# DearCaat/RRT-MIL

Hardware: AMD Instinct MI355X
Metric: slides/sec RRTEncoder fwd, N=9000 D=512 region_num=8 (higher is better)
Workload: dtype f32

## Files before the change

include/rrt_hip.h:

```cpp
#ifndef RRT_HIP_H
#define RRT_HIP_H
#include <stddef.h>
#include <stdint.h>

#ifdef __cplusplus
extern "C" {
#endif

#define RRT_ABI_VERSION 29
#define RRT_MAX_RMSA_LAYERS 8
#define RRT_MAX_CRMSA_K 8

enum {
  RRT_OK = 0,
  RRT_E_INVALID = -1,
  RRT_E_UNSUPPORTED = -2,
  RRT_E_WORKSPACE = -3,
  RRT_E_HANDOVER = -4
};

enum { RRT_COMPUTE_F32 = 0, RRT_COMPUTE_BF16 = 1, RRT_COMPUTE_F16 = 2, RRT_COMPUTE_F32X3 = 3 };
enum { RRT_POS_NONE = 0, RRT_POS_PEG = 1, RRT_POS_PPEG = 2 };
enum { RRT_EPEG_ATTN = 0, RRT_EPEG_VALUE_BF = 1, RRT_EPEG_VALUE_AF = 2 };

enum { RRT_ACT_NONE = 0, RRT_ACT_RELU = 1, RRT_ACT_GELU = 2, RRT_ACT_TANH = 3, RRT_ACT_SIGMOID = 4 };

typedef struct rrt_grid {
  int64_t L;
  int32_t H;
  int32_t s;
  int32_t regions_side;
  int64_t add;
} rrt_grid;

typedef struct rrt_encoder_desc {
  int32_t dim;
  int32_t n_heads;
  int32_t n_rmsa_layers;
  int32_t region_num;
  int32_t region_size;
  int32_t min_region_num;
  float   min_region_ratio;
  int32_t epeg;
  int32_t epeg_k;
  int32_t cr_msa;
  int32_t crmsa_k;
  int32_t crmsa_heads;
  int32_t crmsa_mlp;
  int32_t all_shortcut;
  int32_t compute;
  int32_t ffn;
  int32_t ffn_act;
  int32_t ffn_hidden;
  int32_t pos;
  int32_t pos_pos;
  int32_t peg_k;
  int32_t peg_1d;
  int32_t epeg_2d;
  int32_t epeg_type;
  int32_t weights16_valid;
  int32_t solo;
} rrt_encoder_desc;

typedef struct rrt_attn_weights {
  const float *norm_w, *norm_b;
  const float *qkv_w, *qkv_b;
  const float *proj_w, *proj_b;
  const float *pe_w, *pe_b;
  const float *norm2_w, *norm2_b;
  const float *fc1_w, *fc1_b;
  const float *fc2_w, *fc2_b;
} rrt_attn_weights;

typedef struct rrt_encoder_weights {
  rrt_attn_weights rmsa[RRT_MAX_RMSA_LAYERS];
  rrt_attn_weights crmsa;
  const float *phi;
  const float *phi0_w, *phi2_w;
  const float *norm_w, *norm_b;
  const float *pos_w[3], *pos_b[3];
  uint64_t version;
} rrt_encoder_weights;

int         rrt_abi_version(void);
const char *rrt_strerror(int code);

int rrt_region_grid(int64_t L, int32_t region_num, int32_t region_size,
                    int32_t min_region_num, float min_region_ratio, rrt_grid *out);

int rrt_encoder_workspace_size(const rrt_encoder_desc *desc, int64_t n_tokens, size_t *bytes);

#define RRT_PLAN_FUSED      1
#define RRT_PLAN_FUSED_PROJ 2
#define RRT_PLAN_FUSED16    4
#define RRT_PLAN_FUSED_X3   8
#define RRT_PLAN_CRMSA_PARTS 16
#define RRT_PLAN_ATTN_HD    32
int rrt_encoder_plan(const rrt_encoder_desc *desc, int64_t n_tokens, int32_t *flags);
int rrt_encoder_plan_rows(const rrt_encoder_desc *desc, int64_t n_tokens, int32_t *w);

int rrt_encoder_forward_f32(const rrt_encoder_desc *desc, const rrt_encoder_weights *w,
                            const float *x, float *y, int64_t n_tokens,
                            void *workspace, size_t workspace_bytes, void *stream);

int rrt_debug_encoder_forward_rows_f32(const rrt_encoder_desc *desc, const rrt_encoder_weights *w,
                                       const float *x, float *y, int64_t n_tokens,
                                       void *workspace, size_t workspace_bytes, void *stream, int32_t rows_w);

enum {
  RRT_EV_START = 0,
  RRT_EV_LN_PARTITION,
  RRT_EV_QKV,
  RRT_EV_ATTN,
  RRT_EV_PROJ,
  RRT_EV_CR_COMBINE,
  RRT_EV_CR_INNER,
  RRT_EV_END,
  RRT_EV_COUNT
};
int rrt_encoder_forward_events_f32(const rrt_encoder_desc *desc, const rrt_encoder_weights *w,
                                   const float *x, float *y, int64_t n_tokens,
                                   void *workspace, size_t workspace_bytes, void *stream,
                                   void **events);

typedef struct rrt_phase_gate rrt_phase_gate;
int rrt_phase_gate_create(rrt_phase_gate **out);
int rrt_phase_gate_destroy(rrt_phase_gate *gate);
int rrt_encoder_forward_gated_f32(const rrt_encoder_desc *desc, const rrt_encoder_weights *w,
                                  const float *x, float *y, int64_t n_tokens,
                                  void *workspace, size_t workspace_bytes, void *stream,
                                  rrt_phase_gate *gate, void **events);

int rrt_encoder_batch_workspace_size(const rrt_encoder_desc *desc, int32_t batch, int64_t n_tokens, size_t *bytes);
int rrt_encoder_forward_batch_f32(const rrt_encoder_desc *desc, const rrt_encoder_weights *w,
                                  const float *x, float *y, int32_t batch, int64_t n_tokens,
                                  void *workspace, size_t workspace_bytes, void *stream);


int rrt_ln_partition_f32(const float *x, const float *gamma, const float *beta, float *u,
                         int64_t L, int32_t dim, const rrt_grid *g, void *stream);

int rrt_ln_partition_rows_f32(const float *x, const float *gamma, const float *beta, float *u,
                              int64_t L, int32_t dim, const rrt_grid *g, int32_t w,
                              int32_t *zero, int32_t n_zero, void *stream);

int rrt_linear_f32(const float *A, const float *B, const float *bias, float *C,
                   int64_t M, int32_t N, int32_t K, int32_t q_cols, float q_scale,
                   int32_t compute , void *stream);

int rrt_linear_unpartition_residual_f32(const float *A, const float *B, const float *bias,
                                        const float *resid, float *out, int32_t N, int32_t K,
                                        const rrt_grid *g, int32_t compute, void *stream);

enum { RRT_LINEAR_OPS_F32 = 0, RRT_LINEAR_OPS_16 = 1, RRT_LINEAR_OPS_SPLIT = 2 };
enum { RRT_LINEAR_EPI_PLAIN = 0, RRT_LINEAR_EPI_UNPART = 1, RRT_LINEAR_EPI_ACT = 2, RRT_LINEAR_EPI_UNPART_DROP = 3,
       RRT_LINEAR_EPI_DROP = 4 };
enum { RRT_LINEAR_KERNEL_PLAIN = 0, RRT_LINEAR_KERNEL_WS = 1, RRT_LINEAR_KERNEL_SPLITK = 2 };
#define RRT_LINEAR_PLAN_INTS 12
int rrt_linear_plan(int64_t M, int32_t N, int32_t K, int32_t compute, int32_t operands, int32_t epilogue,
                    int32_t solo, int32_t zero64, int32_t *plan);

int rrt_debug_linear_f32(const void *A, const void *B, const float *bias, const float *resid, float *C,
                         int64_t M, int32_t N, int32_t K, const rrt_grid *g, int32_t operands, int32_t compute,
                         int32_t q_cols, float q_scale, int32_t act, int32_t solo,
                         float drop_p, uint64_t drop_seed, int32_t drop_layer, int32_t *zero64, void *stream);

int rrt_region_attention_f32(const float *qkv, const float *pe_w, float *o,
                             int32_t n_regions, int32_t P, int32_t dim, int32_t heads,
                             int32_t epeg_k, void *stream);

int rrt_region_attention_hd_supported(int32_t P, int32_t dim, int32_t heads, int32_t epeg_k);
int rrt_region_attention_hd_f32(const float *qkv, const float *pe_w, float *o,
                                int32_t n_regions, int32_t P, int32_t dim, int32_t heads,
                                int32_t epeg_k, void *stream);

int rrt_rmsa_fused_f32(const float *u, const float *qkv_w, const float *qkv_b, const float *pe_w,
                       float *o, int32_t n_regions, int32_t P, int32_t dim, int32_t heads,
                       int32_t epeg_k, int32_t compute, void *stream);

int rrt_rmsa_fused_proj_f32(const float *u, const float *qkv_w, const float *qkv_b, const float *pe_w,
                            const float *proj_w, const float *proj_b, const float *resid, float *out,
                            float *o_scratch, int32_t *counters, int32_t dim, int32_t heads, int32_t epeg_k,
                            const rrt_grid *g, void *stream);
int rrt_rmsa_fused_proj_stats_f32(const float *u, const float *qkv_w, const float *qkv_b, const float *pe_w,
                                  const float *proj_w, const float *proj_b, const float *resid, float *out,
                                  float *o_scratch, int32_t *counters, const float *ln2_gamma, const float *phi,
                                  int32_t crmsa_k, float *part, int32_t dim, int32_t heads, int32_t epeg_k,
                                  const rrt_grid *g, void *stream);
int rrt_crmsa_combine_parts_f32(const float *x1, const float *part, const float *gamma, const float *beta,
                                const float *phi, float *wdisp, float *rep, int64_t n_tokens, int32_t dim, int32_t k,
                                const rrt_grid *g8, void *stream);
int rrt_device_error(int32_t clear);
int rrt_debug_rmsa_fused_proj_f32(const float *u, const float *qkv_w, const float *qkv_b, const float *pe_w,
                                  const float *proj_w, const float *proj_b, const float *resid, float *out,
                                  float *o_scratch, int32_t *counters, int32_t dim, int32_t heads, int32_t epeg_k,
                                  const rrt_grid *g, int32_t lag, int32_t spin_limit, int32_t wait_extra, void *stream);

int rrt_cast16(const float *src, uint16_t *dst, int64_t n, int32_t compute, void *stream);
int rrt_ln_partition16(const float *x, const float *gamma, const float *beta, uint16_t *u, int64_t L,
                       int32_t dim, const rrt_grid *g, int32_t compute, void *stream);
int rrt_linear16_f32(const uint16_t *A, const uint16_t *B, const float *bias, const float *resid, float *C,
                     int64_t M, int32_t N, int32_t K, const rrt_grid *g, int32_t compute, void *stream);
int rrt_rmsa_fused16(const uint16_t *u, const uint16_t *qkv_w, const float *qkv_b, const float *pe_w,
                     uint16_t *o, int32_t n_regions, int32_t P, int32_t dim, int32_t heads, int32_t epeg_k,
                     int32_t compute, void *stream);
int rrt_rmsa_pair16_proj(const uint16_t *u, const uint16_t *qkv_w, const float *qkv_b, const float *pe_w,
                         const uint16_t *proj_w, const float *proj_b, const float *resid, float *out, uint16_t *o,
                         int32_t *cnt, int32_t dim, int32_t heads, int32_t epeg_k, const rrt_grid *g, int32_t compute,
                         void *stream);

int rrt_cast_split(const float *src, void *dst, int64_t n, void *stream);
int rrt_ln_partition_split(const float *x, const float *gamma, const float *beta, void *u, int64_t L,
                           int32_t dim, const rrt_grid *g, void *stream);
int rrt_linear_split_f32(const void *A, const void *B, const float *bias, const float *resid, float *C,
                         int64_t M, int32_t N, int32_t K, const rrt_grid *g, void *stream);
int rrt_rmsa_fused_x3(const void *u, const void *qkv_w, const float *qkv_b, const float *pe_w, void *o,
                      int32_t n_regions, int32_t P, int32_t dim, int32_t heads, int32_t epeg_k, void *stream);

int rrt_crmsa_logits_f32(const float *x1, const float *gamma, const float *beta, const float *phi,
                         float *mean_rstd, float *logits, int64_t L, int32_t dim, int32_t k,
                         const rrt_grid *g8, void *stream);
int rrt_crmsa_combine_f32(const float *x1, const float *gamma, const float *beta,
                          const float *mean_rstd, const float *logits, float *wdisp, float *rep,
                          int64_t L, int32_t dim, int32_t k, const rrt_grid *g8, void *stream);
int rrt_crmsa_region_f32(const float *x1, const float *gamma, const float *beta, const float *phi,
                         float *mean_rstd, float *logits, float *wdisp, float *rep,
                         int64_t L, int32_t dim, int32_t k, const rrt_grid *g8, void *stream);
int rrt_crmsa_region4_f32(const float *x1, const float *gamma, const float *beta, const float *phi,
                          float *mean_rstd, float *logits, float *wdisp, float *rep,
                          int64_t L, int32_t dim, int32_t k, const rrt_grid *g8,
                          void *scratch, size_t scratch_bytes, void *stream);
int rrt_crmsa_stream4_f32(const float *x1, const float *gamma, const float *beta, const float *phi,
                          float *mean_rstd, float *logits, float *wdisp, float *rep,
                          int64_t L, int32_t dim, int32_t k, const rrt_grid *g8,
                          void *scratch, size_t scratch_bytes, void *stream);
int rrt_crmsa_dispatch_ln_f32(const float *x1, const float *x0, const float *wdisp,
                              const float *rep2, const float *gamma,
                              const float *beta, float *y, int64_t L, int32_t dim, int32_t k,
                              const rrt_grid *g8, void *stream);
int rrt_crmsa_dispatch_ln_rows_f32(const float *x1, const float *x0, const float *wdisp,
                                   const float *rep2, const float *gamma,
                                   const float *beta, float *y, int64_t L, int32_t dim, int32_t k,
                                   const rrt_grid *g8, int32_t w, uint16_t *y16, int32_t prec16, void *stream);
int rrt_crmsa_mlp_logits_f32(const float *hid, const float *w2, float *logits, int64_t rows,
                             int32_t hdim, int32_t k, void *stream);
int rrt_layernorm_f32(const float *x1, const float *x0, const float *gamma, const float *beta,
                      float *y, int64_t L, int32_t dim, void *stream);

typedef struct rrt_mil_desc {
  rrt_encoder_desc enc;
  int32_t input_dim;
  int32_t emb_act;
  int32_t n_classes;
  int32_t pool_hidden;
  int32_t pool_act;
  int32_t pool_gated;
  int32_t input16;
} rrt_mil_desc;

typedef struct rrt_mil_weights {
  rrt_encoder_weights enc;
  const float *emb_w, *emb_b;
  const float *pool_a_w, *pool_a_b;
  const float *pool_b_w, *pool_b_b;
  const float *pool_c_w, *pool_c_b;
  const float *pred_w, *pred_b;
} rrt_mil_weights;

int rrt_attn_pool_workspace_size(int64_t n_tokens, int32_t dim, int32_t hidden, size_t *bytes);
int rrt_attn_pool_f32(const float *y, const float *hid_a, const float *hid_b, const float *c_w, const float *c_b,
                      float *pooled, float *attn, float *a_raw, int64_t n_tokens, int32_t dim, int32_t hidden,
                      void *workspace, size_t workspace_bytes, void *stream);
int rrt_attn_pool_backward_f32(const float *y, const float *hid_a, const float *hid_b, const float *c_w,
                               const float *attn, const float *pooled, const float *d_pooled,
                               const float *d_attn, const float *d_raw, const float *c_ext, float *dy,
                               float *dhid_a, float *dhid_b, float *dwcb, int64_t n_tokens, int32_t dim,
                               int32_t hidden, void *workspace, size_t workspace_bytes, void *stream);

int rrt_mil_workspace_size(const rrt_mil_desc *desc, int64_t n_tokens, size_t *bytes);
// ... 412 lines not shown
```

rrt-mil_amd/_lib.py:

```python
import ctypes as C
import os

HERE = os.path.dirname(os.path.abspath(__file__))
LIB_PATH = os.path.join(HERE, "librrt_hip.so")

RRT_MAX_RMSA_LAYERS = 8
RRT_MAX_CRMSA_K = 8
ABI_VERSION = 29

_f32p = C.POINTER(C.c_float)


class Grid(C.Structure):
    _fields_ = [("L", C.c_int64), ("H", C.c_int32), ("s", C.c_int32),
                ("regions_side", C.c_int32), ("add", C.c_int64)]


class EncoderDesc(C.Structure):
    _fields_ = [("dim", C.c_int32), ("n_heads", C.c_int32), ("n_rmsa_layers", C.c_int32),
                ("region_num", C.c_int32), ("region_size", C.c_int32), ("min_region_num", C.c_int32),
                ("min_region_ratio", C.c_float), ("epeg", C.c_int32), ("epeg_k", C.c_int32),
                ("cr_msa", C.c_int32), ("crmsa_k", C.c_int32), ("crmsa_heads", C.c_int32),
                ("crmsa_mlp", C.c_int32), ("all_shortcut", C.c_int32), ("compute", C.c_int32),
                ("ffn", C.c_int32), ("ffn_act", C.c_int32), ("ffn_hidden", C.c_int32),
# ... 57 lines not shown
class DsmilWeights(C.Structure):
    _fields_ = [("enc", EncoderWeights)] + [(n, C.c_void_p) for n in (
        "emb_w", "emb_b", "icls_w", "icls_b", "q_w", "q_b", "fcc_w", "fcc_b")]


class BagmilDesc(C.Structure):
    _fields_ = [("enc", EncoderDesc)] + [(n, C.c_int32) for n in (
        "input_dim", "emb_act", "has_rrt", "n_classes", "pool", "pool_hidden", "pool_act", "deconf_k", "deconf_v", "deconf_j")]


class BagmilWeights(C.Structure):
    _fields_ = [("enc", EncoderWeights)] + [(n, C.c_void_p) for n in (
        "emb_w", "emb_b", "a_w", "a_b", "b_w", "b_b", "c_w", "c_b", "cls_w", "cls_b", "conf", "q_w", "q_b", "k_w", "k_b")]


class NystromDesc(C.Structure):
    _fields_ = [(n, C.c_int32) for n in ("dim", "heads", "dim_head", "num_landmarks", "pinv_iterations", "residual",
                                         "residual_conv_kernel")]


NYSTROM_BAG, NYSTROM_REGIONS = 1, 2


class EncoderNystromDesc(C.Structure):
    _fields_ = [("mode", C.c_int32), ("attn", NystromDesc)]


class NystromWeights(C.Structure):
    _fields_ = [(n, C.c_void_p) for n in ("qkv_w", "out_w", "out_b", "conv_w")]


class NystromGrads(C.Structure):
    _fields_ = [(n, C.c_void_p) for n in ("qkv_w", "out_w", "out_b", "conv_w")]


class TransmilDesc(C.Structure):
    _fields_ = [("input_dim", C.c_int32), ("n_classes", C.c_int32), ("act", C.c_int32), ("attn", NystromDesc)]


class TransmilLayerWeights(C.Structure):
    _fields_ = [("norm_w", C.c_void_p), ("norm_b", C.c_void_p), ("attn", NystromWeights)]


class TransmilWeights(C.Structure):
    _fields_ = [("fc1_w", C.c_void_p), ("fc1_b", C.c_void_p), ("cls_token", C.c_void_p), ("layer", TransmilLayerWeights * 2),
                ("pos_w", C.c_void_p * 3), ("pos_b", C.c_void_p * 3), ("norm_w", C.c_void_p), ("norm_b", C.c_void_p),
                ("fc2_w", C.c_void_p), ("fc2_b", C.c_void_p)]


class TransmilLayerGrads(C.Structure):
    _fields_ = [("norm_w", C.c_void_p), ("norm_b", C.c_void_p), ("attn", NystromGrads)]


class TransmilGrads(C.Structure):
    _fields_ = [("fc1_w", C.c_void_p), ("fc1_b", C.c_void_p), ("cls_token", C.c_void_p), ("layer", TransmilLayerGrads * 2),
                ("pos_w", C.c_void_p * 3), ("pos_b", C.c_void_p * 3), ("norm_w", C.c_void_p), ("norm_b", C.c_void_p),
                ("fc2_w", C.c_void_p), ("fc2_b", C.c_void_p)]


class MaskStage(C.Structure):
    _fields_ = [("largest", C.c_int32), ("k", C.c_int64), ("pick", C.c_void_p)]


class Bag(C.Structure):
    _fields_ = [("x", C.c_void_p), ("y", C.c_void_p), ("n_tokens", C.c_int64)]


ACT_NONE, ACT_RELU, ACT_GELU, ACT_TANH, ACT_SIGMOID = 0, 1, 2, 3, 4
ACT_BY_NAME = {"relu": ACT_RELU, "gelu": ACT_GELU, "tanh": ACT_TANH}

_TRANSMIL_FWD_TRAIN = [C.POINTER(TransmilDesc), C.POINTER(TransmilWeights), C.c_void_p, C.c_void_p, C.c_int64, C.c_void_p,
                       C.c_size_t, C.c_float, C.c_float, C.c_uint64, C.c_void_p]
_TRANSMIL_BWD = [C.POINTER(TransmilDesc), C.POINTER(TransmilWeights), C.c_void_p, C.c_void_p, C.c_void_p, C.c_size_t,
                 C.POINTER(TransmilGrads), C.c_void_p, C.c_int64, C.c_void_p, C.c_size_t, C.c_float, C.c_float, C.c_uint64,
                 C.c_void_p]

SIGNATURES = {
    "rrt_abi_version": (C.c_int, []),
    "rrt_strerror": (C.c_char_p, [C.c_int]),
    "rrt_region_grid": (C.c_int, [C.c_int64, C.c_int32, C.c_int32, C.c_int32, C.c_float, C.POINTER(Grid)]),
    "rrt_encoder_workspace_size": (C.c_int, [C.POINTER(EncoderDesc), C.c_int64, C.POINTER(C.c_size_t)]),
    "rrt_encoder_plan": (C.c_int, [C.POINTER(EncoderDesc), C.c_int64, C.POINTER(C.c_int32)]),
    "rrt_encoder_plan_rows": (C.c_int, [C.POINTER(EncoderDesc), C.c_int64, C.POINTER(C.c_int32)]),
    "rrt_encoder_forward_f32": (C.c_int, [C.POINTER(EncoderDesc), C.POINTER(EncoderWeights), C.c_void_p,
                                          C.c_void_p, C.c_int64, C.c_void_p, C.c_size_t, C.c_void_p]),
    "rrt_debug_encoder_forward_rows_f32": (C.c_int, [C.POINTER(EncoderDesc), C.POINTER(EncoderWeights), C.c_void_p,
                                                     C.c_void_p, C.c_int64, C.c_void_p, C.c_size_t, C.c_void_p, C.c_int32]),
    "rrt_encoder_forward_events_f32": (C.c_int, [C.POINTER(EncoderDesc), C.POINTER(EncoderWeights), C.c_void_p,
                                                 C.c_void_p, C.c_int64, C.c_void_p, C.c_size_t, C.c_void_p,
                                                 C.POINTER(C.c_void_p)]),
    "rrt_encoder_batch_workspace_size": (C.c_int, [C.POINTER(EncoderDesc), C.c_int32, C.c_int64, C.POINTER(C.c_size_t)]),
    "rrt_encoder_forward_batch_f32": (C.c_int, [C.POINTER(EncoderDesc), C.POINTER(EncoderWeights), C.c_void_p, C.c_void_p,
                                                C.c_int32, C.c_int64, C.c_void_p, C.c_size_t, C.c_void_p]),
    "rrt_phase_gate_create": (C.c_int, [C.POINTER(C.c_void_p)]),
    "rrt_phase_gate_destroy": (C.c_int, [C.c_void_p]),
    "rrt_encoder_forward_gated_f32": (C.c_int, [C.POINTER(EncoderDesc), C.POINTER(EncoderWeights), C.c_void_p,
                                                C.c_void_p, C.c_int64, C.c_void_p, C.c_size_t, C.c_void_p,
                                                C.c_void_p, C.POINTER(C.c_void_p)]),
    "rrt_ln_partition_f32": (C.c_int, [C.c_void_p, C.c_void_p, C.c_void_p, C.c_void_p, C.c_int64,
                                       C.c_int32, C.POINTER(Grid), C.c_void_p]),
    "rrt_ln_partition_rows_f32": (C.c_int, [C.c_void_p, C.c_void_p, C.c_void_p, C.c_void_p, C.c_int64,
                                            C.c_int32, C.POINTER(Grid), C.c_int32, C.c_void_p, C.c_int32, C.c_void_p]),
    "rrt_linear_f32": (C.c_int, [C.c_void_p, C.c_void_p, C.c_void_p, C.c_void_p, C.c_int64, C.c_int32,
                                 C.c_int32, C.c_int32, C.c_float, C.c_int32, C.c_void_p]),
    "rrt_linear_unpartition_residual_f32": (C.c_int, [C.c_void_p, C.c_void_p, C.c_void_p, C.c_void_p,
                                                      C.c_void_p, C.c_int32, C.c_int32, C.POINTER(Grid),
                                                      C.c_int32, C.c_void_p]),
    "rrt_linear_plan": (C.c_int, [C.c_int64, C.c_int32, C.c_int32, C.c_int32, C.c_int32, C.c_int32, C.c_int32, C.c_int32,
                                  C.POINTER(C.c_int32)]),
    "rrt_debug_linear_f32": (C.c_int, [C.c_void_p] * 5 + [C.c_int64, C.c_int32, C.c_int32, C.POINTER(Grid), C.c_int32,
                                                          C.c_int32, C.c_int32, C.c_float, C.c_int32, C.c_int32, C.c_float,
                                                          C.c_uint64, C.c_int32, C.c_void_p, C.c_void_p]),
    "rrt_region_attention_f32": (C.c_int, [C.c_void_p, C.c_void_p, C.c_void_p, C.c_int32, C.c_int32,
                                           C.c_int32, C.c_int32, C.c_int32, C.c_void_p]),
    "rrt_region_attention_hd_supported": (C.c_int, [C.c_int32] * 4),
    "rrt_region_attention_hd_f32": (C.c_int, [C.c_void_p, C.c_void_p, C.c_void_p, C.c_int32, C.c_int32,
                                              C.c_int32, C.c_int32, C.c_int32, C.c_void_p]),
    "rrt_rmsa_fused_f32": (C.c_int, [C.c_void_p] * 5 + [C.c_int32] * 6 + [C.c_void_p]),
    "rrt_rmsa_fused_proj_f32": (C.c_int, [C.c_void_p] * 10 + [C.c_int32] * 3 + [C.c_void_p] * 2),
    "rrt_device_error": (C.c_int, [C.c_int32]),
    "rrt_rmsa_fused_proj_stats_f32": (C.c_int, [C.c_void_p] * 12 + [C.c_int32, C.c_void_p] + [C.c_int32] * 3 + [C.c_void_p] * 2),
    "rrt_crmsa_combine_parts_f32": (C.c_int, [C.c_void_p] * 7 + [C.c_int64, C.c_int32, C.c_int32, C.POINTER(Grid), C.c_void_p]),
    "rrt_debug_rmsa_fused_proj_f32": (C.c_int, [C.c_void_p] * 10 + [C.c_int32] * 3 + [C.c_void_p] + [C.c_int32] * 3 + [C.c_void_p]),
    "rrt_cast16": (C.c_int, [C.c_void_p, C.c_void_p, C.c_int64, C.c_int32, C.c_void_p]),
    "rrt_ln_partition16": (C.c_int, [C.c_void_p, C.c_void_p, C.c_void_p, C.c_void_p, C.c_int64, C.c_int32,
                                     C.POINTER(Grid), C.c_int32, C.c_void_p]),
    "rrt_linear16_f32": (C.c_int, [C.c_void_p] * 5 + [C.c_int64, C.c_int32, C.c_int32, C.POINTER(Grid), C.c_int32,
                                                      C.c_void_p]),
    "rrt_rmsa_fused16": (C.c_int, [C.c_void_p] * 5 + [C.c_int32] * 6 + [C.c_void_p]),
    "rrt_rmsa_pair16_proj": (C.c_int, [C.c_void_p] * 10 + [C.c_int32] * 3 + [C.POINTER(Grid), C.c_int32, C.c_void_p]),
    "rrt_cast_split": (C.c_int, [C.c_void_p, C.c_void_p, C.c_int64, C.c_void_p]),
    "rrt_ln_partition_split": (C.c_int, [C.c_void_p, C.c_void_p, C.c_void_p, C.c_void_p, C.c_int64, C.c_int32,
                                         C.POINTER(Grid), C.c_void_p]),
    "rrt_linear_split_f32": (C.c_int, [C.c_void_p] * 5 + [C.c_int64, C.c_int32, C.c_int32, C.POINTER(Grid), C.c_void_p]),
    "rrt_rmsa_fused_x3": (C.c_int, [C.c_void_p] * 5 + [C.c_int32] * 5 + [C.c_void_p]),
    "rrt_crmsa_logits_f32": (C.c_int, [C.c_void_p] * 6 + [C.c_int64, C.c_int32, C.c_int32,
                                                         C.POINTER(Grid), C.c_void_p]),
    "rrt_crmsa_combine_f32": (C.c_int, [C.c_void_p] * 7 + [C.c_int64, C.c_int32, C.c_int32,
                                                          C.POINTER(Grid), C.c_void_p]),
    "rrt_crmsa_region_f32": (C.c_int, [C.c_void_p] * 8 + [C.c_int64, C.c_int32, C.c_int32, C.POINTER(Grid), C.c_void_p]),
    "rrt_crmsa_region4_f32": (C.c_int, [C.c_void_p] * 8 + [C.c_int64, C.c_int32, C.c_int32, C.POINTER(Grid), C.c_void_p,
                                                         C.c_size_t, C.c_void_p]),
    "rrt_crmsa_stream4_f32": (C.c_int, [C.c_void_p] * 8 + [C.c_int64, C.c_int32, C.c_int32, C.POINTER(Grid), C.c_void_p,
                                                         C.c_size_t, C.c_void_p]),
    "rrt_crmsa_dispatch_ln_f32": (C.c_int, [C.c_void_p] * 7 + [C.c_int64, C.c_int32, C.c_int32,
                                                              C.POINTER(Grid), C.c_void_p]),
    "rrt_crmsa_dispatch_ln_rows_f32": (C.c_int, [C.c_void_p] * 7 + [C.c_int64, C.c_int32, C.c_int32,
                                                                   C.POINTER(Grid), C.c_int32, C.c_void_p, C.c_int32, C.c_void_p]),
    "rrt_crmsa_mlp_logits_f32": (C.c_int, [C.c_void_p] * 3 + [C.c_int64, C.c_int32, C.c_int32, C.c_void_p]),
    "rrt_layernorm_f32": (C.c_int, [C.c_void_p] * 5 + [C.c_int64, C.c_int32, C.c_void_p]),
    "rrt_peg_f32": (C.c_int, [C.c_void_p] * 4 + [C.c_int64] + [C.c_int32] * 4 + [C.c_void_p]),
    "rrt_peg_backward_workspace_size": (C.c_int, [C.c_int64] + [C.c_int32] * 3 + [C.POINTER(C.c_size_t)]),
    "rrt_peg_backward_f32": (C.c_int, [C.c_void_p] * 6 + [C.c_int64] + [C.c_int32] * 4 + [C.c_void_p, C.c_size_t, C.c_void_p]),
    "rrt_attn_scoremap_scratch_size": (C.c_int, [C.c_int32] * 5 + [C.POINTER(C.c_size_t)]),
    "rrt_attn_scoremap_f32": (C.c_int, [C.c_void_p] * 3 + [C.c_int32] * 5 + [C.c_void_p, C.c_size_t, C.c_void_p]),
    "rrt_attn_scoremap_backward_f32": (C.c_int, [C.c_void_p] * 5 + [C.c_int32] * 5 + [C.c_void_p, C.c_size_t, C.c_void_p]),
    "rrt_value_pe_f32": (C.c_int, [C.c_void_p] * 4 + [C.c_int32] * 7 + [C.c_void_p]),
    "rrt_value_pe_backward_f32": (C.c_int, [C.c_void_p] * 7 + [C.c_int32] * 7 + [C.c_void_p]),
    "rrt_mil_workspace_size": (C.c_int, [C.POINTER(MilDesc), C.c_int64, C.POINTER(C.c_size_t)]),
    "rrt_mil_forward_f32": (C.c_int, [C.POINTER(MilDesc), C.POINTER(MilWeights), C.c_void_p, C.c_void_p,
                                      C.c_void_p, C.c_int32, C.c_void_p, C.c_int64, C.c_void_p, C.c_size_t,
                                      C.c_void_p]),
    "rrt_pool_workspace_size": (C.c_int, [C.c_int64, C.c_int32, C.c_int32, C.c_int32, C.POINTER(C.c_size_t)]),
    "rrt_pool_predict_f32": (C.c_int, [C.c_void_p] * 12 + [C.c_int32, C.c_int64] + [C.c_int32] * 5 +
                             [C.c_void_p, C.c_size_t, C.c_void_p]),
    "rrt_attn_pool_workspace_size": (C.c_int, [C.c_int64, C.c_int32, C.c_int32, C.POINTER(C.c_size_t)]),
    "rrt_attn_pool_f32": (C.c_int, [C.c_void_p] * 8 + [C.c_int64, C.c_int32, C.c_int32, C.c_void_p, C.c_size_t, C.c_void_p]),
    "rrt_attn_pool_backward_f32": (C.c_int, [C.c_void_p] * 14 + [C.c_int64, C.c_int32, C.c_int32, C.c_void_p, C.c_size_t,
                                                                 C.c_void_p]),
    "rrt_branch_pool_workspace_size": (C.c_int, [C.c_int64, C.c_int32, C.c_int32, C.c_int32, C.POINTER(C.c_size_t)]),
    "rrt_branch_pool_f32": (C.c_int, [C.c_void_p] * 8 + [C.c_int64, C.c_int32, C.c_int32, C.c_int32, C.c_void_p, C.c_size_t,
                                                         C.c_void_p]),
    "rrt_branch_pool_backward_f32": (C.c_int, [C.c_void_p] * 12 + [C.c_int64, C.c_int32, C.c_int32, C.c_int32, C.c_void_p,
                                                                   C.c_size_t, C.c_void_p]),
    "rrt_topk_rows_f32": (C.c_int, [C.c_void_p, C.c_void_p, C.c_int32, C.c_int64, C.c_int32, C.c_void_p]),
    "rrt_clam_workspace_size": (C.c_int, [C.POINTER(ClamDesc), C.c_int64, C.POINTER(C.c_size_t)]),
    "rrt_clam_forward_f32": (C.c_int, [C.POINTER(ClamDesc), C.POINTER(ClamWeights)] + [C.c_void_p] * 6 +
                             [C.c_int64, C.c_void_p, C.c_size_t, C.c_void_p]),
    "rrt_instance_max_workspace_size": (C.c_int, [C.c_int64, C.c_int32, C.c_int32, C.POINTER(C.c_size_t)]),
    "rrt_instance_max_f32": (C.c_int, [C.c_void_p] * 6 + [C.c_int64, C.c_int32, C.c_int32, C.c_void_p, C.c_size_t, C.c_void_p]),
    "rrt_dsmil_pool_workspace_size": (C.c_int, [C.c_int64, C.c_int32, C.c_int32, C.c_int32, C.POINTER(C.c_size_t)]),
    "rrt_dsmil_pool_f32": (C.c_int, [C.c_void_p] * 10 + [C.c_int64, C.c_int32, C.c_int32, C.c_int32, C.c_void_p, C.c_size_t,
                                                         C.c_void_p]),
    "rrt_dsmil_workspace_size": (C.c_int, [C.POINTER(DsmilDesc), C.c_int64, C.POINTER(C.c_size_t)]),
    "rrt_dsmil_forward_f32": (C.c_int, [C.POINTER(DsmilDesc), C.POINTER(DsmilWeights)] + [C.c_void_p] * 6 +
                              [C.c_int64, C.c_void_p, C.c_size_t, C.c_void_p]),
    "rrt_bag_mean_workspace_size": (C.c_int, [C.c_int64, C.c_int32, C.c_int32, C.POINTER(C.c_size_t)]),
    "rrt_bag_mean_f32": (C.c_int, [C.c_void_p] * 5 + [C.c_int64, C.c_int32, C.c_int32, C.c_void_p, C.c_size_t, C.c_void_p]),
    "rrt_bag_mean_backward_f32": (C.c_int, [C.c_void_p] * 6 + [C.c_int64, C.c_int32, C.c_int32, C.c_void_p]),
    "rrt_deconf_head_f32": (C.c_int, [C.c_void_p] * 11 + [C.c_int32] * 5 + [C.c_void_p]),
    "rrt_bagmil_workspace_size": (C.c_int, [C.POINTER(BagmilDesc), C.c_int64, C.POINTER(C.c_size_t)]),
    "rrt_bagmil_forward_f32": (C.c_int, [C.POINTER(BagmilDesc), C.POINTER(BagmilWeights), C.c_void_p, C.c_void_p, C.c_void_p,
                                         C.c_int32] + [C.c_void_p] * 4 + [C.c_int64, C.c_void_p, C.c_size_t, C.c_void_p]),
    "rrt_executor_create": (C.c_int, [C.POINTER(EncoderDesc), C.c_int32, C.c_int64, C.POINTER(C.c_void_p)]),
    "rrt_executor_create_on_streams": (C.c_int, [C.POINTER(EncoderDesc), C.c_int32, C.POINTER(C.c_void_p), C.c_int64,
                                                 C.POINTER(C.c_void_p)]),
    "rrt_executor_forward": (C.c_int, [C.c_void_p, C.POINTER(EncoderWeights), C.POINTER(Bag), C.c_int32,
                                       C.c_void_p]),
    "rrt_executor_destroy": (C.c_int, [C.c_void_p]),
    "rrt_region_attention_backward_workspace_size": (C.c_int, [C.c_int32] * 5 + [C.POINTER(C.c_size_t)]),
    "rrt_region_attention_backward_f32": (C.c_int, [C.c_void_p] * 6 + [C.c_int32] * 5 + [C.c_void_p, C.c_size_t,
                                                                                       C.c_void_p]),
    "rrt_layernorm_backward_f32": (C.c_int, [C.c_void_p] * 6 + [C.c_int64, C.c_int32, C.POINTER(Grid), C.c_void_p,
                                                                C.c_size_t, C.c_void_p]),
    "rrt_reduce_partials_f32": (C.c_int, [C.c_void_p] * 3 + [C.c_int32, C.c_int64, C.c_int64] + [C.c_int32] * 4 + [C.c_void_p]),
    "rrt_linear_backward_workspace_size": (C.c_int, [C.c_int64, C.c_int32, C.c_int32, C.POINTER(C.c_size_t)]),
# ... 177 lines not shown
```

rrt-mil_amd/csrc/api.hip:

```cpp
#include <math.h>
#include <stdio.h>
#include <string.h>

#include "api_internal.h"

using namespace rrt_api;

namespace {

thread_local char g_detail[256] = "";

int64_t ceil_sqrt(int64_t n) {
  int64_t r = (int64_t)floor(sqrt((double)n));
  while (r * r > n) --r;
  while ((r + 1) * (r + 1) <= n) ++r;
  return r * r == n ? r : r + 1;
}

struct Workspace {
  float *uo, *qkv, *xa, *xb, *mean_rstd, *logits, *wdisp, *rep, *rep_qkv, *rep_o, *rep2, *v8, *hid;
  float *ffn_ln, *ffn_hid, *xp;
  float* pe_out;
  float* smap;
  uint16_t* w16;
// ... 107 lines not shown
  }
  if (N > (int64_t)4000000) return unsupported("bag larger than 4e6 tokens");
  if (d->compute < 0 || d->compute > RRT_COMPUTE_F32X3) return unsupported("compute must be RRT_COMPUTE_F32/BF16/F16/F32X3");
  return RRT_OK;
}

int region_grids(const rrt_encoder_desc* d, int64_t N, rrt_grid* g, rrt_grid* g8) {
  *g = rrt_grid{};
  if (d->n_rmsa_layers > 0) {
    int rc = rrt_region_grid(N, d->region_num, d->region_size, d->min_region_num, d->min_region_ratio, g);
    if (rc) return rc;
  }
  return rrt_region_grid(N, 8, 0, 0, 0.f, g8);
}
int resolve_grids(const rrt_encoder_desc* d, int64_t N, rrt_grid* g, rrt_grid* g8) {
  int rc = check_desc(d, N);
  return rc ? rc : region_grids(d, N, g, g8);
}

GridDev identity_grid(int64_t N) {
  GridDev g{};
  const int Hs = (int)ceil_sqrt(N);
  g.L = (int)N;
  g.H = g.s = Hs;
  g.rs = 1;
  g.P = g.Np = Hs * Hs;
  g.inv_H = g.inv_s = 1.0f / (float)Hs;
  g.inv_rs = 1.0f;
  g.inv_P = 1.0f / (float)g.P;
  g.Rt = 1;
  return g;
}

LinearEpilogue qkv_epilogue(const float* bias, int dim, int heads, int prec) {
  LinearEpilogue ep{};
  ep.prec = prec;
  ep.bias = bias;
  ep.q_cols = dim;
  ep.q_scale = 1.0f / sqrtf((float)(dim / heads));
  return ep;
}

LinearEpilogue proj_epilogue(const float* bias, const float* resid, const GridDev& g, int prec) {
  LinearEpilogue ep{};
  ep.prec = prec;
  ep.bias = bias;
  ep.resid = resid;
  ep.g = g;
  return ep;
}

hipError_t inner_attention(const float* u, int n_regions, int P, const rrt_attn_weights& w, int dim,
                           int heads, int epeg_k, float* qkv, float* o, int prec, bool solo, hipStream_t st) {
  const int M = n_regions * P;
  LinearEpilogue ep = qkv_epilogue(w.qkv_b, dim, heads, prec);
  ep.solo = solo;
  hipError_t e = launch_linear(u, w.qkv_w, qkv, M, 3 * dim, dim, ep, st);
  if (e != hipSuccess) return e;
  return launch_region_attention(qkv, epeg_k > 0 ? w.pe_w : nullptr, o, n_regions, P, dim, heads,
                                 epeg_k, st);
}

enum class LayerKind {
  Pair16Merged,
  Fused16,
  FusedX3,
  EpegVariant,
  FusedProj,
  Fused,
  Unfused,
};
enum class FrontKind { None, Mlp, Parts, RegionInFlight, Region4, Region, Stream4, TwoKernel };
enum class CastKind { None, Images16, Split };
struct EncoderPlan {
  LayerKind layer;
  bool parts;
  bool gated;
  bool attn_hd;
  CastKind casts;
  bool inner16;
  FrontKind front;
  int rows_w;
  bool rows_ln1;
};

constexpr int ROWS_W_DEFAULT = 1;

#ifndef RRT_STREAM4_MIN_P
#define RRT_STREAM4_MIN_P 145
#endif

EncoderPlan plan_encoder(const rrt_encoder_desc& d, const rrt_grid& g, const rrt_grid& g8, bool stops_before_crmsa) {
  EncoderPlan p{};
  p.layer = LayerKind::Unfused;
  const int D = d.dim;
  const bool want_x3 = d.compute == RRT_COMPUTE_F32X3;
  const int compute = want_x3 ? RRT_COMPUTE_F32 : d.compute;
  const bool lowp = compute != RRT_COMPUTE_F32 && D % 64 == 0;
  const GridDev gd8 = to_dev(g8);
  p.inner16 = d.cr_msa && lowp && rmsa_fused16_supported(64, D, d.crmsa_heads, 0);
  {
    static const char* rows_env = rrt_tune_env("RRT_ROWS_W");
    static const bool rows_lowp = rrt_tune_env("RRT_ROWS_LOWP") != nullptr;
    int w = ROWS_W_DEFAULT;
    if (rows_env != nullptr && atoi(rows_env) >= 0 && atoi(rows_env) <= ROWS_W_MAX) w = atoi(rows_env);
    const bool exact = d.compute == RRT_COMPUTE_F32;
    const bool fits = D <= 512 && (!d.cr_msa || d.crmsa_k <= 3);
    if (!d.solo && fits && (exact || (rows_lowp && lowp))) {
      p.rows_w = w;
      p.rows_ln1 = exact && w > 0;
    }
  }
  if (d.n_rmsa_layers > 0) {
    const GridDev gd = to_dev(g);
    const int R = gd.rs * gd.rs, heads = d.n_heads, ek = d.epeg ? d.epeg_k : 0;
    const bool rows_ok = rmsa_fused_supported_rows(gd.Np, D);
    static const bool want_merged16 = rrt_tune_env("RRT_PAIR16_PROJ") != nullptr;
    if (d.epeg && (d.epeg_2d || d.epeg_type != RRT_EPEG_ATTN)) {
      p.layer = LayerKind::EpegVariant;
    } else if (lowp && rmsa_fused16_supported(gd.P, D, heads, ek) && rows_ok) {
      p.layer = want_merged16 && rmsa_pair16_proj_supported(R, gd.P, D, heads, ek) ? LayerKind::Pair16Merged : LayerKind::Fused16;
    } else if (want_x3 && D % 256 == 0 && rmsa_fused_x3_supported(gd.P, D, heads, ek) && rows_ok) {
      p.layer = LayerKind::FusedX3;
    } else if (compute == RRT_COMPUTE_F32 && rows_ok && rmsa_fused_proj_supported(R, gd.P, D, heads, ek, compute)) {
      p.layer = LayerKind::FusedProj;
      p.parts = d.solo != 0 && d.cr_msa && !d.crmsa_mlp && !d.ffn && d.crmsa_k <= 4 && !stops_before_crmsa && D % 64 == 0 &&
                crmsa_combine_parts_supported(D, d.crmsa_k, gd8);
    } else if (rmsa_fused_supported(gd.P, D, heads, ek) && rows_ok) {
      p.layer = LayerKind::Fused;
    } else {
      p.attn_hd = region_attention_hd_supported(gd.P, D, heads, ek);
    }
    p.gated = gd.P > 112 && p.layer != LayerKind::EpegVariant && p.layer != LayerKind::Unfused;
    if (p.layer != LayerKind::EpegVariant) p.casts = lowp ? CastKind::Images16 : want_x3 ? CastKind::Split : CastKind::None;
  }
  if (!d.cr_msa || stops_before_crmsa) return p;
  const int k = d.crmsa_k;
  const bool has_counters = d.n_rmsa_layers > 0;
  static const bool no_region_inflight = rrt_tune_env("RRT_NO_REGION_INFLIGHT") != nullptr;
  static const bool region_lowp = rrt_tune_env("RRT_REGION_INFLIGHT_LOWP") != nullptr;
  if (d.crmsa_mlp) {
    p.front = FrontKind::Mlp;
  } else if (p.parts) {
    p.front = FrontKind::Parts;
  } else if (!no_region_inflight && !d.solo && p.layer != LayerKind::FusedX3 && (compute == RRT_COMPUTE_F32 || region_lowp) &&
             crmsa_region_supported(D, k, gd8)) {
    p.front = FrontKind::RegionInFlight;
  } else if (has_counters && crmsa_region4_supported(D, k, gd8) && gd8.P < RRT_STREAM4_MIN_P) {
    p.front = FrontKind::Region4;
  } else if (crmsa_region_enabled() && crmsa_region_supported(D, k, gd8)) {
    p.front = FrontKind::Region;
  } else if (has_counters && gd8.P >= RRT_STREAM4_MIN_P && crmsa_stream4_supported(D, k, gd8)) {
    p.front = FrontKind::Stream4;
  } else {
    p.front = FrontKind::TwoKernel;
  }
  return p;
}

}

GridDev to_dev(const rrt_grid& g) {
  GridDev d;
  d.L = (int)g.L;
  d.H = g.H;
  d.s = g.s;
  d.rs = g.regions_side;
  d.P = g.s * g.s;
  d.Np = g.H * g.H;
  d.inv_H = 1.0f / (float)d.H;
  d.inv_s = 1.0f / (float)d.s;
  d.inv_rs = 1.0f / (float)d.rs;
  d.inv_P = 1.0f / (float)d.P;
  d.Rt = d.rs * d.rs;
  return d;
}

extern "C" {

int rrt_abi_version(void) { return RRT_ABI_VERSION; }

const char* rrt_strerror(int code) {
  switch (code) {
    case RRT_OK: return "ok";
    case RRT_E_INVALID: return "invalid argument (null pointer or non-positive size)";
    case RRT_E_UNSUPPORTED: return g_detail[0] ? g_detail : "unsupported configuration";
    case RRT_E_WORKSPACE: return "workspace too small (see rrt_encoder_workspace_size)";
    case RRT_E_HANDOVER: return "an earlier merged R-MSA launch gave up its in-launch hand-over wait; outputs in flight are invalid "
                                "(synchronise, then rrt_device_error(1) to clear)";
    default: return code > 0 ? hipGetErrorString((hipError_t)code) : "unknown error";
  }
}

int rrt_region_grid(int64_t L, int32_t region_num, int32_t region_size, int32_t min_region_num,
                    float min_region_ratio, rrt_grid* out) {
  if (!out || L <= 0) return RRT_E_INVALID;
  if (region_size <= 0 && region_num <= 0) return RRT_E_INVALID;
  int64_t H = ceil_sqrt(L), s;
  if (region_size > 0) {
    H += ((-H) % region_size + region_size) % region_size;
    s = region_size;
  } else {
    H += ((-H) % region_num + region_num) % region_num;
    s = H / region_num;
  }
  int64_t add = H * H - L;
  if ((double)add > (double)L / ((double)min_region_ratio + 1e-8) || L < min_region_num) {
    H = ceil_sqrt(L);
    H += H % 2;
    add = H * H - L;
    s = H;
  }
  if (H > 46340) return RRT_E_INVALID;
  out->L = L;
  out->H = (int32_t)H;
  out->s = (int32_t)s;
  out->regions_side = (int32_t)(H / s);
  out->add = add;
  return RRT_OK;
}

int rrt_encoder_workspace_size(const rrt_encoder_desc* desc, int64_t n_tokens, size_t* bytes) {
  if (!bytes) return RRT_E_INVALID;
  rrt_grid g{}, g8{};
  int rc = resolve_grids(desc, n_tokens, &g, &g8);
  if (rc) return rc;
  *bytes = carve(*desc, n_tokens, g, g8, nullptr).bytes;
  return RRT_OK;
}

int rrt_encoder_plan(const rrt_encoder_desc* desc, int64_t n_tokens, int32_t* flags) {
  if (!flags) return RRT_E_INVALID;
  *flags = 0;
  rrt_grid g{}, g8{};
  int rc = resolve_grids(desc, n_tokens, &g, &g8);
  if (rc) return rc;
  if (desc->n_rmsa_layers <= 0) return RRT_OK;
  const EncoderPlan plan = plan_encoder(*desc, g, g8, false);
  switch (plan.layer) {
    case LayerKind::Pair16Merged:
    case LayerKind::Fused16: *flags = RRT_PLAN_FUSED16; break;
    case LayerKind::FusedX3: *flags = RRT_PLAN_FUSED_X3; break;
    case LayerKind::FusedProj: *flags = RRT_PLAN_FUSED | RRT_PLAN_FUSED_PROJ | (plan.parts ? RRT_PLAN_CRMSA_PARTS : 0); break;
    case LayerKind::Fused: *flags = RRT_PLAN_FUSED; break;
    case LayerKind::Unfused: *flags = plan.attn_hd ? RRT_PLAN_ATTN_HD : 0; break;
    case LayerKind::EpegVariant: break;
  }
  return RRT_OK;
}

int rrt_encoder_plan_rows(const rrt_encoder_desc* desc, int64_t n_tokens, int32_t* w) {
  if (!w) return RRT_E_INVALID;
  *w = 0;
  rrt_grid g{}, g8{};
  int rc = resolve_grids(desc, n_tokens, &g, &g8);
  if (rc) return rc;
  *w = plan_encoder(*desc, g, g8, false).rows_w;
  return RRT_OK;
}

struct rrt_phase_gate {
  hipEvent_t done;
  bool armed;
};

static int ffn_apply(const rrt_encoder_desc* desc, const rrt_attn_weights& lw, const float* xi, float* xo,
                     const Workspace& ws, int64_t N, hipStream_t st) {
  if (!lw.norm2_w || !lw.norm2_b || !lw.fc1_w || !lw.fc1_b || !lw.fc2_w || !lw.fc2_b) return RRT_E_INVALID;
  const int D = desc->dim;
  RRT_TRY(launch_layernorm(xi, nullptr, lw.norm2_w, lw.norm2_b, ws.ffn_ln, (int)N, D, st));
  LinearEpilogue e1{};
  e1.prec = desc->compute;
  e1.bias = lw.fc1_b;
  e1.act = desc->ffn_act;
  RRT_TRY(launch_linear(ws.ffn_ln, lw.fc1_w, ws.ffn_hid, (int)N, desc->ffn_hidden, D, e1, st));
  return (int)launch_linear(ws.ffn_hid, lw.fc2_w, xo, (int)N, D, desc->ffn_hidden,
                            proj_epilogue(lw.fc2_b, xi, identity_grid(N), desc->compute), st);
}

static int encoder_forward(const rrt_encoder_desc* desc_in, const rrt_encoder_weights* w, const float* x,
                           float* y, int64_t n_tokens, void* workspace, size_t workspace_bytes,
                           void* stream, void** events, rrt_phase_gate* gate = nullptr, float* rmsa_out = nullptr,
                           uint16_t* y16 = nullptr, bool* y16_done = nullptr, int rows_w_forced = -1,
                           const float* shortcut = nullptr) {
  if (y16_done) *y16_done = false;
  if (!desc_in || !w || !x || !y || x == y) return RRT_E_INVALID;
  int rc = check_desc(desc_in, n_tokens);
  if (rc) return rc;
  if (handover_err_peek(false)) return RRT_E_HANDOVER;
  rrt_grid g{}, g8{};
  rc = region_grids(desc_in, n_tokens, &g, &g8);
  if (rc) return rc;
  rrt_encoder_desc dloc = *desc_in;
  if (dloc.compute == RRT_COMPUTE_F32X3) dloc.compute = RRT_COMPUTE_F32;
  const rrt_encoder_desc* const desc = &dloc;
  hipStream_t st = (hipStream_t)stream;
  const int D = desc->dim;
  const int64_t N = n_tokens;
  Workspace ws = carve(*desc, N, g, g8, nullptr);
  if (!workspace || workspace_bytes < ws.bytes) return RRT_E_WORKSPACE;
  ws = carve(*desc, N, g, g8, (char*)workspace);
  EncoderPlan plan = plan_encoder(*desc_in, g, g8, rmsa_out != nullptr);
  if (rows_w_forced >= 0) {
    plan.rows_w = rows_w_forced;
    plan.rows_ln1 = rows_w_forced > 0 && desc_in->compute == RRT_COMPUTE_F32;
  }

  auto mark = [&](int i) -> hipError_t {
    return (events && events[i]) ? hipEventRecord((hipEvent_t)events[i], st) : hipSuccess;
  };
  RRT_TRY(mark(RRT_EV_START));

  auto ffn_block = [&](const rrt_attn_weights& lw, const float* xi, float* xo) -> int {
    return ffn_apply(desc, lw, xi, xo, ws, N, st);
  };

  const float* xin = x;
  auto pos_embed = [&]() -> int {
    if (!w->pos_w[0] || (desc->pos == RRT_POS_PPEG && (!w->pos_w[1] || !w->pos_w[2]))) return RRT_E_INVALID;
    RRT_TRY(launch_peg(xin, w->pos_w, w->pos_b, ws.xp, (int)N, D, desc->peg_k, desc->peg_1d, desc->pos == RRT_POS_PPEG, st));
    xin = ws.xp;
    return RRT_OK;
  };
  if (desc->pos && desc->pos_pos == -1) {
    rc = pos_embed();
    if (rc) return rc;
  }
  {
    const bool split = plan.casts == CastKind::Split;
    const size_t per_w = split ? 2 : 1;
    Cast16Jobs jobs{};
    if (plan.casts != CastKind::None) {
      for (int li = 0; li < desc->n_rmsa_layers; ++li) {
        const rrt_attn_weights& lw = w->rmsa[li];
        if (!lw.qkv_w || !lw.proj_w) return RRT_E_INVALID;
        uint16_t* base = ws.w16 + (size_t)li * per_w * 4 * D * D;
        jobs.add(lw.qkv_w, base, (size_t)3 * D * D);
        jobs.add(lw.proj_w, base + per_w * 3 * D * D, (size_t)D * D);
      }
    }
    if (plan.inner16) {
      if (!w->crmsa.qkv_w || !w->crmsa.proj_w) return RRT_E_INVALID;
      jobs.add(w->crmsa.qkv_w, ws.wcr16, (size_t)3 * D * D);
      jobs.add(w->crmsa.proj_w, ws.wcr16 + (size_t)3 * D * D, (size_t)D * D);
    }
    if (jobs.count && !desc->weights16_valid) RRT_TRY(split ? launch_cast_split(jobs, st) : launch_cast16(jobs, desc->compute, st));
  }
  rrt_phase_gate* const gt = (gate && plan.gated) ? gate : nullptr;
  auto gate_record = [&]() -> hipError_t {
    if (!gt) return hipSuccess;
    const hipError_t ge = hipEventRecord(gt->done, st);
    if (ge == hipSuccess) gt->armed = true;
    return ge;
  };
  auto core_begin = [&](bool marks) -> hipError_t {
    if (gt && gt->armed) {
      const hipError_t ge = hipStreamWaitEvent(st, gt->done, 0);
      if (ge != hipSuccess) return ge;
    }
    return marks ? mark(RRT_EV_LN_PARTITION) : hipSuccess;
  };
  auto core_end = [&](bool marks, bool record = true) -> hipError_t {
    hipError_t ge = record ? gate_record() : hipSuccess;
    if (ge == hipSuccess && marks) ge = mark(RRT_EV_QKV);
    if (ge == hipSuccess && marks) ge = mark(RRT_EV_ATTN);
    return ge;
  };
  static const bool gate_proj = rrt_tune_env("RRT_GATE_PROJ") != nullptr;
  for (int li = 0; li < desc->n_rmsa_layers; ++li) {
    if (li == 1 && desc->pos && desc->pos_pos == 0) {
      rc = pos_embed();
      if (rc) return rc;
    }
    const rrt_attn_weights& lw = w->rmsa[li];
    const bool last = li == desc->n_rmsa_layers - 1;
    if (!lw.norm_w || !lw.norm_b || !lw.qkv_w || !lw.proj_w || !lw.proj_b) return RRT_E_INVALID;
    if (desc->epeg && !lw.pe_w) return RRT_E_INVALID;
    if (plan.parts && last && (!w->crmsa.norm_w || !w->crmsa.norm_b || !w->phi)) return RRT_E_INVALID;
    const GridDev gd = to_dev(g);
    const int R = gd.rs * gd.rs, ek = desc->epeg ? desc->epeg_k : 0;
    const float* const pe_w = desc->epeg ? lw.pe_w : nullptr;
    const bool to_out = rmsa_out != nullptr && last;
    float* xout = desc->ffn ? ws.xa : (to_out ? rmsa_out : ((li & 1) ? ws.xb : ws.xa));
    float* const fout = to_out ? rmsa_out : ws.xb;
    const bool marks = li == 0 && plan.layer != LayerKind::EpegVariant;
    auto out_ep = [&](int prec) {
      LinearEpilogue ep = proj_epilogue(lw.proj_b, xin, gd, prec);
      ep.zero64 = ws.cr_cnt;
      return ep;
    };
    switch (plan.layer) {
      case LayerKind::Pair16Merged:
      case LayerKind::Fused16: {
        const bool merged16 = plan.layer == LayerKind::Pair16Merged;
        uint16_t* u16 = (uint16_t*)ws.uo;
        uint16_t* o16 = (uint16_t*)ws.qkv;
        const uint16_t* wq16 = ws.w16 + (size_t)li * 4 * D * D;
        RRT_TRY(launch_ln_partition16(xin, lw.norm_w, lw.norm_b, u16, D, gd, desc->compute, st, merged16 ? ws.proj_cnt : nullptr,
                                      merged16 ? R / 2 : 0));
        RRT_TRY(core_begin(marks));
        if (merged16) {
          PairProj pj{};
          pj.Wp = wq16 + (size_t)3 * D * D;
          pj.bias = lw.proj_b;
          pj.resid = xin;
          pj.out = xout;
          pj.cnt = ws.proj_cnt;
          pj.zero64 = ws.cr_cnt;
          pj.g = gd;
          RRT_TRY(launch_rmsa_pair16_proj(u16, wq16, lw.qkv_b, pe_w, o16, R, gd.P, D, desc->n_heads, ek, desc->compute, pj, st));
          RRT_TRY(core_end(marks));
        } else {
          RRT_TRY(launch_rmsa_fused16(u16, wq16, lw.qkv_b, pe_w, o16, R, gd.P, D, desc->n_heads, ek, desc->compute, st));
          RRT_TRY(core_end(marks));
          LinearEpilogue ep = out_ep(desc->compute);
          ep.solo = desc->solo != 0;
          RRT_TRY(launch_linear16(o16, wq16 + (size_t)3 * D * D, xout, gd.Np, D, D, ep, st));
        }
        break;
      }
      case LayerKind::FusedX3: {
        const uint16_t* wq = ws.w16 + (size_t)li * 8 * D * D;
        RRT_TRY(launch_ln_partition_split(xin, lw.norm_w, lw.norm_b, ws.uo, D, gd, st));
        RRT_TRY(core_begin(marks));
        RRT_TRY(launch_rmsa_fused_x3(ws.uo, wq, lw.qkv_b, pe_w, ws.qkv, R, gd.P, D, desc->n_heads, ek, st));
        RRT_TRY(core_end(marks));
        RRT_TRY(launch_linear_split(ws.qkv, wq + (size_t)6 * D * D, xout, gd.Np, D, D, out_ep(0), st));
        break;
      }
      case LayerKind::FusedProj: {
        RRT_TRY(launch_ln_partition(xin, lw.norm_w, lw.norm_b, ws.uo, D, gd, st, ws.proj_cnt, R, plan.rows_ln1 ? plan.rows_w : 0));
        RRT_TRY(core_begin(marks));
        FusedProj pj{};
        pj.Wp = lw.proj_w;
        pj.bias = lw.proj_b;
        pj.resid = xin;
        pj.out = xout;
        pj.cnt = ws.proj_cnt;
        pj.zero64 = ws.cr_cnt;
        pj.g = gd;
        if (plan.parts && last) {
          pj.part = ws.cr_pstat;
          pj.ln_g = w->crmsa.norm_w;
          pj.phi = w->phi;
          pj.k = desc->crmsa_k;
        }
        RRT_TRY(launch_rmsa_fused(ws.uo, lw.qkv_w, lw.qkv_b, pe_w, ws.qkv, R, gd.P, D, desc->n_heads, ek, desc->compute, st,
                                  nullptr, &pj));
        RRT_TRY(core_end(marks));
        break;
      }
      case LayerKind::Fused: {
        RRT_TRY(launch_ln_partition(xin, lw.norm_w, lw.norm_b, ws.uo, D, gd, st, nullptr, 0, plan.rows_ln1 ? plan.rows_w : 0));
        RRT_TRY(core_begin(marks));
        RRT_TRY(launch_rmsa_fused(ws.uo, lw.qkv_w, lw.qkv_b, pe_w, ws.qkv, R, gd.P, D, desc->n_heads, ek, desc->compute, st));
        RRT_TRY(core_end(marks, !gate_proj));
        RRT_TRY(launch_linear(ws.qkv, lw.proj_w, xout, gd.Np, D, D, out_ep(desc->compute), st));
        if (gate_proj) RRT_TRY(gate_record());
        break;
      }
      case LayerKind::Unfused: {
        RRT_TRY(launch_ln_partition(xin, lw.norm_w, lw.norm_b, ws.uo, D, gd, st, nullptr, 0, plan.rows_ln1 ? plan.rows_w : 0));
        RRT_TRY(core_begin(marks));
        RRT_TRY(launch_linear(ws.uo, lw.qkv_w, ws.qkv, gd.Np, 3 * D, D, qkv_epilogue(lw.qkv_b, D, desc->n_heads, desc->compute), st));
        if (marks) RRT_TRY(mark(RRT_EV_QKV));
        RRT_TRY(launch_region_attention(ws.qkv, pe_w, ws.uo, R, gd.P, D, desc->n_heads, ek, st));
        if (marks) RRT_TRY(mark(RRT_EV_ATTN));
        RRT_TRY(launch_linear(ws.uo, lw.proj_w, xout, gd.Np, D, D, out_ep(desc->compute), st));
        break;
      }
      case LayerKind::EpegVariant: {
        RRT_TRY(launch_ln_partition(xin, lw.norm_w, lw.norm_b, ws.uo, D, gd, st));
        RRT_TRY(launch_linear(ws.uo, lw.qkv_w, ws.qkv, gd.Np, 3 * D, D, qkv_epilogue(lw.qkv_b, D, desc->n_heads, desc->compute), st));
        if (desc->epeg_type == RRT_EPEG_ATTN) {
          RRT_TRY(launch_attn_scoremap(ws.qkv, lw.pe_w, ws.uo, ws.smap, R, gd.P, D, desc->n_heads, desc->epeg_k, st));
        } else {
          RRT_TRY(launch_value_pe(ws.qkv, lw.pe_w, lw.pe_b, ws.pe_out, R, gd.P, gd.s, D, desc->n_heads, desc->epeg_k,
                                  desc->epeg_2d, st));
          if (desc->epeg_type == RRT_EPEG_VALUE_BF)
            RRT_TRY(launch_add_cols(ws.qkv + 2 * D, ws.pe_out, (size_t)gd.Np, D, 3 * D, st));
          RRT_TRY(launch_region_attention(ws.qkv, nullptr, ws.uo, R, gd.P, D, desc->n_heads, 0, st));
          if (desc->epeg_type == RRT_EPEG_VALUE_AF)
            RRT_TRY(launch_add_cols(ws.uo, ws.pe_out, (size_t)gd.Np, D, D, st));
        }
        RRT_TRY(launch_linear(ws.uo, lw.proj_w, xout, gd.Np, D, D, out_ep(desc->compute), st));
        break;
      }
    }
    if (marks) RRT_TRY(mark(RRT_EV_PROJ));
    xin = xout;
    if (desc->ffn) {
      rc = ffn_block(lw, xout, fout);
      if (rc) return rc;
      xin = fout;
    }
  }
  if (rmsa_out != nullptr) {
    if (xin != rmsa_out) RRT_TRY(hipMemcpyAsync(rmsa_out, xin, (size_t)N * D * sizeof(float), hipMemcpyDeviceToDevice, st));
    return RRT_OK;
  }
  const float* x0 = desc->all_shortcut ? (shortcut ? shortcut : x) : nullptr;
  if (!w->norm_w || !w->norm_b) return RRT_E_INVALID;
  if (!desc->cr_msa) {
    RRT_TRY(launch_layernorm(xin, x0, w->norm_w, w->norm_b, y, (int)N, D, st, plan.rows_w));
    RRT_TRY(mark(RRT_EV_END));
    return RRT_OK;
  }
  const rrt_attn_weights& cw = w->crmsa;
  if (!cw.norm_w || !cw.norm_b || !cw.qkv_w || !cw.proj_w || !cw.proj_b) return RRT_E_INVALID;
  if (desc->crmsa_mlp ? (!w->phi0_w || !w->phi2_w) : !w->phi) return RRT_E_INVALID;
  const GridDev gd8 = to_dev(g8);
  const int k = desc->crmsa_k, R8 = gd8.rs * gd8.rs;
  uint16_t* const rep16 = plan.inner16 ? ws.rep16 : nullptr;
  switch (plan.front) {
    case FrontKind::Mlp: {
      RRT_TRY(launch_ln_partition(xin, cw.norm_w, cw.norm_b, ws.v8, D, gd8, st));
      LinearEpilogue ep{};
      ep.prec = desc->compute;
      RRT_TRY(launch_linear(ws.v8, w->phi0_w, ws.hid, gd8.Np, D / 4, D, ep, st));
      RRT_TRY(launch_crmsa_mlp_logits(ws.hid, w->phi2_w, ws.logits, gd8.Np, D / 4, k, st));
      RRT_TRY(launch_crmsa_combine(ws.v8, nullptr, nullptr, nullptr, ws.logits, ws.wdisp, ws.rep, rep16, desc->compute, D, k, gd8, st));
      break;
    }
    case FrontKind::Parts:
      RRT_TRY(launch_crmsa_combine_parts(xin, ws.cr_pstat, cw.norm_w, cw.norm_b, w->phi, ws.wdisp, ws.rep, rep16, desc->compute, D,
                                         k, gd8, st));
      break;
    case FrontKind::RegionInFlight:
      RRT_TRY(launch_crmsa_region(xin, cw.norm_w, cw.norm_b, w->phi, nullptr, nullptr, ws.wdisp, ws.rep, k, gd8, st, rep16,
                                  desc->compute));
      break;
    case FrontKind::Region4:
      RRT_TRY(launch_crmsa_region4(xin, cw.norm_w, cw.norm_b, w->phi, nullptr, ws.logits, ws.wdisp, ws.rep, rep16, desc->compute,
                                   ws.cr_part, ws.cr_cnt, k, gd8, st));
      break;
    case FrontKind::Region:
      RRT_TRY(launch_crmsa_region(xin, cw.norm_w, cw.norm_b, w->phi, nullptr, nullptr, ws.wdisp, ws.rep, k, gd8, st));
      break;
    case FrontKind::Stream4:
      RRT_TRY(launch_crmsa_stream4(xin, cw.norm_w, cw.norm_b, w->phi, nullptr, ws.logits, ws.wdisp, ws.rep, rep16, desc->compute,
                                   ws.cr_part, ws.cr_cnt, k, gd8, st));
      break;
    case FrontKind::TwoKernel:
      RRT_TRY(launch_crmsa_logits(xin, cw.norm_w, cw.norm_b, w->phi, ws.mean_rstd, ws.logits, D, k, gd8, st));
      RRT_TRY(launch_crmsa_combine(xin, cw.norm_w, cw.norm_b, ws.mean_rstd, ws.logits, ws.wdisp, ws.rep, rep16, desc->compute, D, k,
                                   gd8, st));
      break;
    case FrontKind::None: break;
  }
  RRT_TRY(mark(RRT_EV_CR_COMBINE));
  if (plan.inner16) {
    if (plan.front == FrontKind::Region) {
      Cast16Jobs cj{};
      cj.add(ws.rep, ws.rep16, (size_t)k * R8 * D);
      RRT_TRY(launch_cast16(cj, desc->compute, st));
    }
    RRT_TRY(launch_rmsa_fused16(ws.rep16, ws.wcr16, cw.qkv_b, nullptr, ws.repo16, k, R8, D, desc->crmsa_heads, 0,
                                desc->compute, st));
    LinearEpilogue ep{};
    ep.prec = desc->compute;
    ep.bias = cw.proj_b;
    RRT_TRY(launch_linear16(ws.repo16, ws.wcr16 + (size_t)3 * D * D, ws.rep2, k * R8, D, D, ep, st));
  } else {
    static const bool inner_solo = rrt_tune_env("RRT_INNER_SOLO") != nullptr;
    RRT_TRY(inner_attention(ws.rep, k, R8, cw, D, desc->crmsa_heads, 0, ws.rep_qkv, ws.rep_o, desc->compute, desc->solo != 0 || inner_solo, st));
    LinearEpilogue ep{};
    ep.prec = desc->compute;
    ep.bias = cw.proj_b;
    ep.solo = desc->solo != 0 || inner_solo;
    RRT_TRY(launch_linear(ws.rep_o, cw.proj_w, ws.rep2, k * R8, D, D, ep, st));
  }
  RRT_TRY(mark(RRT_EV_CR_INNER));
  if (desc->ffn) {
    RRT_TRY(launch_crmsa_dispatch_ln(xin, nullptr, ws.wdisp, ws.rep2, nullptr, nullptr, ws.xa, D, k, gd8, st, nullptr, 0, plan.rows_w));
    rc = ffn_block(cw, ws.xa, ws.xb);
    if (rc) return rc;
    RRT_TRY(launch_layernorm(ws.xb, x0, w->norm_w, w->norm_b, y, (int)N, D, st, plan.rows_w));
    RRT_TRY(mark(RRT_EV_END));
    return RRT_OK;
  }
  const bool want16 = y16 != nullptr && (desc->compute == RRT_COMPUTE_BF16 || desc->compute == RRT_COMPUTE_F16) && D % 4 == 0;
  RRT_TRY(launch_crmsa_dispatch_ln(xin, x0, ws.wdisp, ws.rep2, w->norm_w, w->norm_b, y, D, k,
                                   gd8, st, want16 ? y16 : nullptr, want16 ? desc->compute : 0, plan.rows_w));
  if (want16 && y16_done) *y16_done = true;
  RRT_TRY(mark(RRT_EV_END));
  return RRT_OK;
}

int rrt_encoder_forward_f32(const rrt_encoder_desc* desc, const rrt_encoder_weights* w, const float* x,
                            float* y, int64_t n_tokens, void* workspace, size_t workspace_bytes,
                            void* stream) {
  return encoder_forward(desc, w, x, y, n_tokens, workspace, workspace_bytes, stream, nullptr);
}

int rrt_debug_encoder_forward_rows_f32(const rrt_encoder_desc* desc, const rrt_encoder_weights* w, const float* x, float* y,
                                       int64_t n_tokens, void* workspace, size_t workspace_bytes, void* stream, int32_t rows_w) {
  if (rows_w < 0 || rows_w > ROWS_W_MAX) return RRT_E_INVALID;
  return encoder_forward(desc, w, x, y, n_tokens, workspace, workspace_bytes, stream, nullptr, nullptr, nullptr, nullptr, nullptr,
                         rows_w);
}

}

namespace rrt_api {
static rrt_encoder_desc tail_desc(const rrt_encoder_desc* desc) {
  rrt_encoder_desc t = *desc;
  t.n_rmsa_layers = 0;
  t.pos = RRT_POS_NONE;
  t.weights16_valid = 0;
  return t;
}
int encoder_tail_workspace_size(const rrt_encoder_desc* desc, int64_t n_tokens, size_t* bytes) {
  const rrt_encoder_desc t = tail_desc(desc);
  return rrt_encoder_workspace_size(&t, n_tokens, bytes);
}
int encoder_tail(const rrt_encoder_desc* desc, const rrt_encoder_weights* w, const float* x1, const float* x0, float* y,
                 int64_t n_tokens, void* workspace, size_t workspace_bytes, void* stream) {
  const rrt_encoder_desc t = tail_desc(desc);
  return encoder_forward(&t, w, x1, y, n_tokens, workspace, workspace_bytes, stream, nullptr, nullptr, nullptr, nullptr, nullptr,
                         -1, x0);
}
}

extern "C" {
int rrt_phase_gate_create(rrt_phase_gate** out) {
  if (!out) return RRT_E_INVALID;
  rrt_phase_gate* g = new rrt_phase_gate();
  g->armed = false;
  hipError_t e = hipEventCreateWithFlags(&g->done, hipEventDisableTiming);
  if (e != hipSuccess) {
    delete g;
    return (int)e;
  }
  *out = g;
  return RRT_OK;
}

int rrt_phase_gate_destroy(rrt_phase_gate* g) {
  if (!g) return RRT_OK;
  (void)hipEventDestroy(g->done);
  delete g;
  return RRT_OK;
}

int rrt_encoder_forward_gated_f32(const rrt_encoder_desc* desc, const rrt_encoder_weights* w, const float* x,
                                  float* y, int64_t n_tokens, void* workspace, size_t workspace_bytes,
                                  void* stream, rrt_phase_gate* gate, void** events) {
  return encoder_forward(desc, w, x, y, n_tokens, workspace, workspace_bytes, stream, events, gate);
}

int rrt_encoder_forward_events_f32(const rrt_encoder_desc* desc, const rrt_encoder_weights* w,
                                   const float* x, float* y, int64_t n_tokens, void* workspace,
                                   size_t workspace_bytes, void* stream, void** events) {
  return encoder_forward(desc, w, x, y, n_tokens, workspace, workspace_bytes, stream, events);
}

namespace {
struct BatchWs {
  Workspace one;
  float *x1, *mean_rstd, *logits, *wdisp, *rep, *rep_qkv, *rep_o, *rep2;
  size_t one_bytes, bytes;
};
BatchWs carve_batch(const rrt_encoder_desc& d, int64_t B, int64_t N, const rrt_grid& g, const rrt_grid& g8, char* base) {
  BatchWs w{};
  w.one_bytes = carve(d, N, g, g8, nullptr).bytes;
  Arena a{base};
  w.one = carve(d, N, g, g8, a.take<char>(w.one_bytes));
  const size_t D = d.dim, Np8 = (size_t)g8.H * g8.H, R8 = (size_t)g8.regions_side * g8.regions_side, k = d.crmsa_k;
  w.x1 = a.take((size_t)B * N * D);
  if (d.cr_msa) {
    w.mean_rstd = a.take((size_t)B * N * 2);
    w.logits = a.take((size_t)B * Np8 * k);
    w.wdisp = a.take((size_t)B * Np8 * k);
    w.rep = a.take(k * R8 * B * D);
    w.rep_qkv = a.take(k * R8 * B * 3 * D);
    w.rep_o = a.take(k * R8 * B * D);
    w.rep2 = a.take(k * R8 * B * D);
// ... 106 lines not shown
int rrt_ln_partition_rows_f32(const float* x, const float* gamma, const float* beta, float* u, int64_t L,
                              int32_t dim, const rrt_grid* g, int32_t w, int32_t* zero, int32_t n_zero, void* stream) {
  if (!x || !gamma || !beta || !u || !g || L != g->L || dim <= 0 || dim % 4) return RRT_E_INVALID;
  if (w < 0 || w > ROWS_W_MAX || n_zero < 0 || (n_zero > 0 && !zero)) return RRT_E_INVALID;
  if (dim > 2048) return unsupported("dim > 2048");
  return (int)launch_ln_partition(x, gamma, beta, u, dim, to_dev(*g), (hipStream_t)stream, n_zero > 0 ? zero : nullptr, n_zero, w);
}

int rrt_linear_f32(const float* A, const float* B, const float* bias, float* C, int64_t M, int32_t N,
                   int32_t K, int32_t q_cols, float q_scale, int32_t compute, void* stream) {
  if (!A || !B || !C || M <= 0 || N <= 0 || K <= 0) return RRT_E_INVALID;
  if (K % 32) return unsupported("linear: K must be a multiple of 32");
  if (compute < 0 || compute > 2) return unsupported("compute must be RRT_COMPUTE_F32/BF16/F16");
  LinearEpilogue ep{};
  ep.prec = compute;
  ep.bias = bias;
  ep.q_cols = q_cols;
  ep.q_scale = q_scale;
  return (int)launch_linear(A, B, C, (int)M, N, K, ep, (hipStream_t)stream);
}

int rrt_linear_unpartition_residual_f32(const float* A, const float* B, const float* bias,
                                        const float* resid, float* out, int32_t N, int32_t K,
                                        const rrt_grid* g, int32_t compute, void* stream) {
  if (!A || !B || !resid || !out || !g || N <= 0 || K <= 0) return RRT_E_INVALID;
  if (K % 32) return unsupported("linear: K must be a multiple of 32");
  if (compute < 0 || compute > 2) return unsupported("compute must be RRT_COMPUTE_F32/BF16/F16");
  const LinearEpilogue ep = proj_epilogue(bias, resid, to_dev(*g), compute);
  return (int)launch_linear(A, B, out, ep.g.Np, N, K, ep, (hipStream_t)stream);
}

int rrt_region_attention_f32(const float* qkv, const float* pe_w, float* o, int32_t n_regions, int32_t P,
                             int32_t dim, int32_t heads, int32_t epeg_k, void* stream) {
  if (!qkv || !o || n_regions <= 0 || P <= 0 || dim <= 0 || heads <= 0 || dim % heads) return RRT_E_INVALID;
  if (pe_w && epeg_k > 0 && epeg_k % 2 == 0) return unsupported("epeg_k must be odd");
  return (int)launch_region_attention(qkv, pe_w, o, n_regions, P, dim, heads, epeg_k, (hipStream_t)stream);
}

int rrt_region_attention_hd_supported(int32_t P, int32_t dim, int32_t heads, int32_t epeg_k) {
  return region_attention_hd_supported(P, dim, heads, epeg_k) ? 1 : 0;
}

int rrt_region_attention_hd_f32(const float* qkv, const float* pe_w, float* o, int32_t n_regions, int32_t P, int32_t dim,
                                int32_t heads, int32_t epeg_k, void* stream) {
  if (n_regions <= 0 || P <= 0 || dim <= 0 || heads <= 0 || dim % heads) return RRT_E_INVALID;
  const int ek = pe_w ? epeg_k : 0;
  if (!region_attention_hd_supported(P, dim, heads, ek))
    return unsupported("region_attention_hd: needs a head dim that is a multiple of 16 in [16, 256] other than 64 and "
                       "epeg_k <= 63 (use rrt_region_attention_f32)");
  if (!qkv || !o) return RRT_E_INVALID;
  if (ek > 0 && ek % 2 == 0) return unsupported("epeg_k must be odd");
  if (n_regions > 65535) return unsupported("region_attention_hd: more than 65535 regions in one call");
  return (int)launch_region_attention_hd(qkv, pe_w, o, n_regions, P, dim, heads, ek, (hipStream_t)stream);
}

int rrt_rmsa_fused_f32(const float* u, const float* qkv_w, const float* qkv_b, const float* pe_w, float* o,
                       int32_t n_regions, int32_t P, int32_t dim, int32_t heads, int32_t epeg_k,
                       int32_t compute, void* stream) {
  if (!u || !qkv_w || !o || n_regions <= 0 || P <= 0 || dim <= 0 || heads <= 0) return RRT_E_INVALID;
  if (compute < 0 || compute > 2) return unsupported("compute must be RRT_COMPUTE_F32/BF16/F16");
  const int ek = pe_w ? epeg_k : 0;
  if (!rmsa_fused_supported(P, dim, heads, ek) || !rmsa_fused_supported_rows((long)n_regions * P, dim))
    return unsupported("rmsa_fused: needs head dim 64, 48 < P <= 208, epeg_k <= 63 (use linear + region_attention)");
  return (int)launch_rmsa_fused(u, qkv_w, qkv_b, pe_w, o, n_regions, P, dim, heads, ek, compute,
                                (hipStream_t)stream);
}

int rrt_device_error(int32_t clear) { return handover_err_peek(clear != 0); }

int rrt_rmsa_fused_proj_f32(const float* u, const float* qkv_w, const float* qkv_b, const float* pe_w,
                            const float* proj_w, const float* proj_b, const float* resid, float* out, float* o_scratch,
                            int32_t* counters, int32_t dim, int32_t heads, int32_t epeg_k, const rrt_grid* g,
                            void* stream) {
  return rrt_debug_rmsa_fused_proj_f32(u, qkv_w, qkv_b, pe_w, proj_w, proj_b, resid, out, o_scratch, counters, dim, heads,
                                       epeg_k, g, 0, 0, 0, stream);
}

}

static int fused_proj_stage(const float* u, const float* qkv_w, const float* qkv_b, const float* pe_w,
                            const float* proj_w, const float* proj_b, const float* resid, float* out, float* o_scratch,
                            int32_t* counters, int32_t dim, int32_t heads, int32_t epeg_k, const rrt_grid* g,
                            int32_t lag, int32_t spin_limit, int32_t wait_extra, const float* ln2_gamma, const float* phi,
                            int32_t crmsa_k, float* part, void* stream) {
  if (!u || !qkv_w || !proj_w || !resid || !out || !o_scratch || !counters || !g || dim <= 0 || heads <= 0 || out == resid ||
      lag < 0 || spin_limit < 0 || wait_extra < 0)
    return RRT_E_INVALID;
  if (handover_err_peek(false)) return RRT_E_HANDOVER;
  const GridDev gd = to_dev(*g);
  const int ek = pe_w ? epeg_k : 0, R = gd.rs * gd.rs;
  if (!rmsa_fused_proj_supported(R, gd.P, dim, heads, ek, RRT_COMPUTE_F32) || !rmsa_fused_supported_rows(gd.Np, dim))
    return unsupported("rmsa_fused_proj: needs what rmsa_fused needs (head dim 64, 64 < P <= 208, epeg_k <= 63) and at "
                       "least two rounds of (region, head) items (heads * regions >= 2 x the CU count)");
  RRT_TRY(hipMemsetAsync(counters, 0, (size_t)R * sizeof(int32_t), (hipStream_t)stream));
  FusedProj pj{};
  pj.Wp = proj_w;
  pj.bias = proj_b;
  pj.resid = resid;
  pj.out = out;
  pj.cnt = counters;
  pj.g = gd;
  pj.lag = lag;
  pj.spin_limit = spin_limit;
  pj.wait_for = wait_extra > 0 ? heads + wait_extra : 0;
  pj.part = part;
  pj.ln_g = ln2_gamma;
  pj.phi = phi;
  pj.k = crmsa_k;
  if (lag > 0 && (lag < 8 * heads || lag > heads * R)) return unsupported("rmsa_fused_proj: lag must be in [8 * heads, heads * regions]");
  return (int)launch_rmsa_fused(u, qkv_w, qkv_b, pe_w, o_scratch, R, gd.P, dim, heads, ek, RRT_COMPUTE_F32,
                                (hipStream_t)stream, nullptr, &pj);
}

extern "C" {

int rrt_debug_rmsa_fused_proj_f32(const float* u, const float* qkv_w, const float* qkv_b, const float* pe_w,
                                  const float* proj_w, const float* proj_b, const float* resid, float* out, float* o_scratch,
                                  int32_t* counters, int32_t dim, int32_t heads, int32_t epeg_k, const rrt_grid* g,
                                  int32_t lag, int32_t spin_limit, int32_t wait_extra, void* stream) {
  return fused_proj_stage(u, qkv_w, qkv_b, pe_w, proj_w, proj_b, resid, out, o_scratch, counters, dim, heads, epeg_k, g, lag,
                          spin_limit, wait_extra, nullptr, nullptr, 0, nullptr, stream);
}

int rrt_rmsa_fused_proj_stats_f32(const float* u, const float* qkv_w, const float* qkv_b, const float* pe_w,
                                  const float* proj_w, const float* proj_b, const float* resid, float* out, float* o_scratch,
                                  int32_t* counters, const float* ln2_gamma, const float* phi, int32_t crmsa_k, float* part,
                                  int32_t dim, int32_t heads, int32_t epeg_k, const rrt_grid* g, void* stream) {
  if (!ln2_gamma || !phi || !part || crmsa_k < 1 || crmsa_k > RRT_MAX_CRMSA_K) return RRT_E_INVALID;
  return fused_proj_stage(u, qkv_w, qkv_b, pe_w, proj_w, proj_b, resid, out, o_scratch, counters, dim, heads, epeg_k, g, 0, 0, 0,
                          ln2_gamma, phi, crmsa_k, part, stream);
}

int rrt_crmsa_combine_parts_f32(const float* x1, const float* part, const float* gamma, const float* beta, const float* phi,
                                float* wdisp, float* rep, int64_t n_tokens, int32_t dim, int32_t k, const rrt_grid* g8,
                                void* stream) {
  if (!x1 || !part || !gamma || !beta || !phi || !wdisp || !rep || !g8 || n_tokens <= 0 || g8->L != n_tokens) return RRT_E_INVALID;
  const GridDev gd = to_dev(*g8);
  if (!crmsa_combine_parts_supported(dim, k, gd)) return unsupported("crmsa_combine_parts: dim % 64 == 0, dim <= 512, 1 <= k <= 8");
  return (int)launch_crmsa_combine_parts(x1, part, gamma, beta, phi, wdisp, rep, nullptr, 0, dim, k, gd, (hipStream_t)stream);
}

int rrt_cast16(const float* src, uint16_t* dst, int64_t n, int32_t compute, void* stream) {
  if (!src || !dst || n <= 0 || n % 4) return RRT_E_INVALID;
  if (compute != RRT_COMPUTE_BF16 && compute != RRT_COMPUTE_F16) return unsupported("cast16: compute must be BF16 or F16");
  Cast16Jobs jobs{};
  jobs.add(src, dst, (size_t)n);
  return (int)launch_cast16(jobs, compute, (hipStream_t)stream);
}

int rrt_ln_partition16(const float* x, const float* gamma, const float* beta, uint16_t* u, int64_t L, int32_t dim,
                       const rrt_grid* g, int32_t compute, void* stream) {
  if (!x || !gamma || !beta || !u || !g || L != g->L || dim <= 0 || dim % 4) return RRT_E_INVALID;
  if (dim > 2048) return unsupported("dim > 2048");
  if (compute != RRT_COMPUTE_BF16 && compute != RRT_COMPUTE_F16) return unsupported("compute must be BF16 or F16");
  return (int)launch_ln_partition16(x, gamma, beta, u, dim, to_dev(*g), compute, (hipStream_t)stream);
}

int rrt_linear16_f32(const uint16_t* A, const uint16_t* B, const float* bias, const float* resid, float* C, int64_t M,
                     int32_t N, int32_t K, const rrt_grid* g, int32_t compute, void* stream) {
  if (!A || !B || !C || M <= 0 || N <= 0 || K <= 0 || (resid && !g)) return RRT_E_INVALID;
  if (K % 64) return unsupported("linear16: K must be a multiple of 64");
  if (compute != RRT_COMPUTE_BF16 && compute != RRT_COMPUTE_F16) return unsupported("compute must be BF16 or F16");
  LinearEpilogue ep{};
  ep.prec = compute;
  ep.bias = bias;
  if (resid) {
    ep.resid = resid;
    ep.g = to_dev(*g);
    if (M != ep.g.Np) return RRT_E_INVALID;
  }
  return (int)launch_linear16(A, B, C, (int)M, N, K, ep, (hipStream_t)stream);
}

int rrt_rmsa_fused16(const uint16_t* u, const uint16_t* qkv_w, const float* qkv_b, const float* pe_w, uint16_t* o,
                     int32_t n_regions, int32_t P, int32_t dim, int32_t heads, int32_t epeg_k, int32_t compute,
                     void* stream) {
  if (!u || !qkv_w || !o || n_regions <= 0 || P <= 0 || dim <= 0 || heads <= 0) return RRT_E_INVALID;
  if (compute != RRT_COMPUTE_BF16 && compute != RRT_COMPUTE_F16) return unsupported("compute must be BF16 or F16");
  const int ek = pe_w ? epeg_k : 0;
  if (!rmsa_fused16_supported(P, dim, heads, ek) || !rmsa_fused_supported_rows((long)n_regions * P, dim))
    return unsupported("rmsa_fused16: needs head dim 64, 16 < P <= 256, epeg_k <= 63");
  return (int)launch_rmsa_fused16(u, qkv_w, qkv_b, pe_w, o, n_regions, P, dim, heads, ek, compute, (hipStream_t)stream);
}

int rrt_rmsa_pair16_proj(const uint16_t* u, const uint16_t* qkv_w, const float* qkv_b, const float* pe_w, const uint16_t* proj_w,
                         const float* proj_b, const float* resid, float* out, uint16_t* o, int32_t* cnt, int32_t dim,
                         int32_t heads, int32_t epeg_k, const rrt_grid* g, int32_t compute, void* stream) {
  if (!u || !qkv_w || !proj_w || !resid || !out || !o || !cnt || !g || dim <= 0 || heads <= 0) return RRT_E_INVALID;
  if (compute != RRT_COMPUTE_BF16 && compute != RRT_COMPUTE_F16) return unsupported("compute must be BF16 or F16");
  if (handover_err_peek(false)) return RRT_E_HANDOVER;
  const GridDev gd = to_dev(*g);
  const int ek = pe_w ? epeg_k : 0, R = gd.rs * gd.rs;
  if (!rmsa_pair16_proj_supported(R, gd.P, dim, heads, ek))
    return unsupported("rmsa_pair16_proj: head dim 64, regions of 65..96 or 113..128 tokens, a multiple of 16 regions, "
                       "at least two rounds of (pair, head) items");
  RRT_TRY(hipMemsetAsync(cnt, 0, (size_t)(R / 2) * sizeof(int), (hipStream_t)stream));
  PairProj pj{};
  pj.Wp = proj_w;
  pj.bias = proj_b;
  pj.resid = resid;
  pj.out = out;
  pj.cnt = cnt;
  pj.g = gd;
  return (int)launch_rmsa_pair16_proj(u, qkv_w, qkv_b, pe_w, o, R, gd.P, dim, heads, ek, compute, pj, (hipStream_t)stream);
}

int rrt_cast_split(const float* src, void* dst, int64_t n, void* stream) {
  if (!src || !dst || n <= 0 || n % 32) return RRT_E_INVALID;
  Cast16Jobs jobs{};
  jobs.add(src, (uint16_t*)dst, (size_t)n);
  return (int)launch_cast_split(jobs, (hipStream_t)stream);
}

// ... 1929 lines not shown
```

rrt-mil_amd/csrc/internal.h:

```cpp
#pragma once
#include <hip/hip_runtime.h>
#include "common.h"
#include "../../include/rrt_hip.h"

GridDev to_dev(const rrt_grid& g);

#ifdef RRT_TUNING
#include <stdlib.h>
inline const char* rrt_tune_env(const char* name) { return getenv(name); }
#else
inline const char* rrt_tune_env(const char*) { return nullptr; }
#endif

struct OncePerDevice {
  bool seen[64] = {};
  bool first() {
    int d = 0;
    (void)hipGetDevice(&d);
    d &= 63;
    if (seen[d]) return false;
    seen[d] = true;
    return true;
  }
};
// ... 33 lines not shown
  int mode;
  int prec;
};
hipError_t plan_linear(int ops, int M, int N, int K, const LinearEpilogue& ep, LinearPlan* out);

constexpr int CAST16_MAX_JOBS = 2 * RRT_MAX_RMSA_LAYERS + 2;
struct Cast16Jobs {
  const float* src[CAST16_MAX_JOBS];
  uint16_t* dst[CAST16_MAX_JOBS];
  size_t n4[CAST16_MAX_JOBS];
  int count;
  void add(const float* s, uint16_t* d, size_t n_elems) {
    src[count] = s;
    dst[count] = d;
    n4[count++] = n_elems / 4;
  }
};
static_assert(sizeof(Cast16Jobs) == 440, "Cast16Jobs is a kernel argument: three 18-entry tables of 8 bytes and the count");
hipError_t launch_cast16(const Cast16Jobs& jobs, int prec, hipStream_t st);
hipError_t launch_ln_partition16(const float* x, const float* gamma, const float* beta, uint16_t* u, int dim,
                                 const GridDev& g, int prec, hipStream_t st, int* zero = nullptr, int n_zero = 0);
hipError_t launch_cast_split(const Cast16Jobs& jobs, hipStream_t st);
hipError_t launch_ln_partition_split(const float* x, const float* gamma, const float* beta, void* u, int dim,
                                     const GridDev& g, hipStream_t st);
hipError_t launch_linear_split(const void* Asplit, const void* Bsplit, float* C, int M, int N, int K,
                               const LinearEpilogue& ep, hipStream_t st);
bool rmsa_pair16_supported(int n_regions, int P, int D, int heads, int epeg_k);
hipError_t launch_rmsa_pair16(const uint16_t* U, const uint16_t* W, const float* bqkv, const float* pe_w, uint16_t* O,
                              int n_regions, int P, int D, int heads, int epeg_k, int prec, hipStream_t st);
struct PairProj {
  const uint16_t* Wp;
  const float* bias;
  const float* resid;
  float* out;
  int* cnt;
  int* zero64;
  int lag;
  int n_items;
  GridDev g;
  int* err;
  int spin_limit;
  int wait_for;
};
bool rmsa_pair16_proj_supported(int n_regions, int P, int D, int heads, int epeg_k);
hipError_t launch_rmsa_pair16_proj(const uint16_t* U, const uint16_t* W, const float* bqkv, const float* pe_w, uint16_t* O,
                                   int n_regions, int P, int D, int heads, int epeg_k, int prec, const PairProj& proj,
                                   hipStream_t st);
bool rmsa_fused_x3_supported(int P, int D, int heads, int epeg_k);
hipError_t launch_rmsa_fused_x3(const void* Usplit, const void* Wsplit, const float* bqkv, const float* pe_w,
                                void* Osplit, int n_regions, int P, int D, int heads, int epeg_k, hipStream_t st);
hipError_t launch_linear16(const void* A16, const void* B16, float* C, int M, int N, int K, const LinearEpilogue& ep,
                           hipStream_t st);
bool rmsa_fused16_supported(int P, int D, int heads, int epeg_k);
hipError_t launch_rmsa_fused16(const uint16_t* U16, const uint16_t* Wqkv16, const float* bqkv, const float* pe_w,
                               uint16_t* O16, int n_regions, int P, int D, int heads, int epeg_k, int prec,
                               hipStream_t st);

hipError_t launch_region_attention(const float* qkv, const float* pe_w, float* o, int n_regions,
                                   int P, int dim, int heads, int epeg_k, hipStream_t st);
bool region_attention_hd_supported(int P, int dim, int heads, int epeg_k);
hipError_t launch_region_attention_hd(const float* qkv, const float* pe_w, float* o, int n_regions, int P, int dim,
                                      int heads, int epeg_k, hipStream_t st);

bool rmsa_fused_supported(int P, int D, int heads, int epeg_k);
bool rmsa_fused_supported_rows(long n_rows, int D);
struct FusedProj {
  const float* Wp;
  const float* bias;
  const float* resid;
  float* out;
  int* cnt;
  int* zero64;
  int lag;
  int n_items;
  GridDev g;
  int* err;
  int spin_limit;
  int wait_for;
  float* part;
  const float* ln_g;
  const float* phi;
  int k;
  int n_slabs;
};
int* handover_err_device();
int handover_err_peek(bool clear);
bool rmsa_fused_proj_supported(int n_regions, int P, int D, int heads, int epeg_k, int prec);
hipError_t launch_rmsa_fused(const float* U, const float* Wqkv, const float* bqkv, const float* pe_w,
                             float* O, int n_regions, int P, int D, int heads, int epeg_k, int prec,
                             hipStream_t st, float* stash = nullptr,
                             const FusedProj* proj = nullptr);

size_t attn_scoremap_lds(int P, int k);
size_t attn_scoremap_scratch_floats(int n_regions, int P, int heads, int k, int maps);
hipError_t launch_attn_scoremap(const float* qkv, const float* pe_w, float* o, float* smap, int n_regions, int P, int dim,
                                int heads, int k, hipStream_t st);
hipError_t launch_value_pe(const float* qkv, const float* w, const float* bias, float* pe, int n_regions, int P, int s,
                           int dim, int heads, int k, int two_d, hipStream_t st);
hipError_t launch_add_cols(float* dst, const float* src, size_t rows, int dim, int ld, hipStream_t st);
hipError_t launch_value_pe_backward(const float* dpe, const float* qkv, const float* vsub, const float* w, float* dqkv, float* dw,
                                    float* db, int n_regions, int P, int s, int dim, int heads, int k, int two_d,
                                    hipStream_t st);
hipError_t launch_copy_cols(float* dst, const float* src, size_t rows, int dim, int ld, int off, hipStream_t st);
hipError_t launch_sub(float* dst, const float* a, const float* b, size_t n, hipStream_t st);
hipError_t launch_small_k_matmul(const float* A, const float* W, float* Cm, int M, int N, int Kd, hipStream_t st);
hipError_t launch_attn_scoremap_backward(const float* qkv, const float* pe_w, const float* dO, float* dqkv, float* dpe_w,
                                         float* scratch, int n_regions, int P, int dim, int heads, int k, hipStream_t st);

hipError_t launch_crmsa_logits(const float* x1, const float* gamma, const float* beta,
                               const float* phi, float* mean_rstd, float* logits, int dim, int k,
                               const GridDev& g8, hipStream_t st);
bool crmsa_region_supported(int dim, int k, const GridDev& g8);
bool crmsa_region_enabled();
bool crmsa_region4_supported(int dim, int k, const GridDev& g8);
size_t crmsa_region4_scratch_floats(const GridDev& g8, int k);
hipError_t launch_crmsa_region4(const float* x1, const float* gamma, const float* beta, const float* phi,
                                float* mean_rstd, float* logits, float* wdisp, float* rep, uint16_t* rep16, int prec16,
                                float* part_g, int* counters, int k, const GridDev& g8, hipStream_t st);
hipError_t launch_crmsa_region(const float* x1, const float* gamma, const float* beta, const float* phi,
                               float* mean_rstd, float* logits, float* wdisp, float* rep, int k, const GridDev& g8,
                               hipStream_t st, uint16_t* rep16 = nullptr, int prec16 = 0);
bool crmsa_stream4_supported(int dim, int k, const GridDev& g8);
hipError_t launch_crmsa_stream4(const float* x1, const float* gamma, const float* beta, const float* phi,
                                float* mean_rstd, float* logits, float* wdisp, float* rep, uint16_t* rep16, int prec16,
                                float* part_g, int* counters, int k, const GridDev& g8, hipStream_t st);
hipError_t launch_crmsa_combine(const float* x1, const float* gamma, const float* beta,
                                const float* mean_rstd, const float* logits, float* wdisp,
                                float* rep, uint16_t* rep16, int prec16, int dim, int k, const GridDev& g8, hipStream_t st);
bool crmsa_combine_parts_supported(int dim, int k, const GridDev& g8);
size_t crmsa_parts_floats(long n_tokens, int dim, int k);
hipError_t launch_crmsa_combine_parts(const float* x1, const float* part, const float* gamma, const float* beta,
                                      const float* phi, float* wdisp, float* rep, uint16_t* rep16, int prec16, int dim,
                                      int k, const GridDev& g8, hipStream_t st);
hipError_t launch_crmsa_mlp_logits(const float* hid, const float* w2, float* logits, int rows, int hdim,
                                   int k, hipStream_t st);
hipError_t launch_crmsa_dispatch_ln(const float* x1, const float* x0, const float* wdisp,
                                    const float* rep2, const float* gamma,
                                    const float* beta, float* y, int dim, int k, const GridDev& g8,
                                    hipStream_t st, uint16_t* y16 = nullptr, int prec16 = 0,
                                    int rows_w = 0);
hipError_t launch_layernorm(const float* x1, const float* x0, const float* gamma,
                            const float* beta, float* y, int L, int dim, hipStream_t st, int rows_w = 0);

constexpr int POOL_CHUNK = 32;
hipError_t launch_pool_partial(const float* y, const float* hid_a, const float* hid_b, const float* wc,
                               const float* bc, float* a_raw, float* part, int N, int dim, int hid,
                               hipStream_t st);
hipError_t launch_pool_merge(const float* part, const float* a_raw, const float* pred_w, const float* pred_b,
                             float* pooled, float* logits, float* attn, int no_norm, int N, int dim,
                             int n_classes, hipStream_t st);

bool pool_merge_fits(int64_t N, int dim);
bool pool_backward_fits(int dim, int hid);

size_t pool_backward_part_floats(int N, int hid);
hipError_t launch_pool_backward(const float* y, const float* hid_a, const float* hid_b, const float* wc, const float* attn,
                                const float* pooled, const float* d_pooled, const float* d_attn, const float* d_raw,
                                const float* c_ext, float* dy, float* dhid_a, float* dhid_b, float* dwcb, float* part, int N,
                                int dim, int hid, hipStream_t st);

size_t branch_pool_part_floats(int N, int dim, int K);
size_t branch_pool_backward_part_floats(int N, int hid, int K);
size_t branch_pool_merge_lds(int N, int dim);
size_t branch_pool_backward_lds(int dim, int hid, int K);
hipError_t launch_branch_pool(const float* y, const float* hid_a, const float* hid_b, const float* wc, const float* bc,
                              const float* cls_w, const float* cls_b, float* pooled, float* logits, float* attn, float* a_raw,
// ... 183 lines not shown
```

rrt-mil_amd/csrc/rmsa_fused.hip:

```cpp
#include <stdio.h>
#include <stdlib.h>
#include <string.h>
#include <mutex>

#include "internal.h"

namespace {

constexpr int BK = 32;
constexpr int HD = 64;
constexpr int BN = 3 * HD;
constexpr float NEG_BIG = -3.0e38f;
constexpr float LOG2E = 1.4426950408889634f;

typedef float f32x2 __attribute__((ext_vector_type(2)));
template <bool WT>
__device__ __forceinline__ void store_o(f32x2* p, f32x2 v) {
  if constexpr (WT) asm volatile("global_store_dwordx2 %0, %1, off sc0 sc1" ::"v"(p), "v"(v) : "memory");
  else *p = v;
}
#define RRT_STORE_O(ptr, val) store_o<PROJ>((ptr), (val))

template <bool WT>
__device__ __forceinline__ void store_o(f32x4* p, f32x4 v) {
  if constexpr (WT) asm volatile("global_store_dwordx4 %0, %1, off sc0 sc1\n\ts_nop 1" ::"v"(p), "v"(v) : "memory");
  else *p = v;
}

typedef __bf16 bf16x8 __attribute__((ext_vector_type(8)));
typedef _Float16 f16x8 __attribute__((ext_vector_type(8)));
enum { PREC_F32 = 0, PREC_BF16 = 1, PREC_F16 = 2 };

template <int PREC>
struct Frag8;
template <>
struct Frag8<PREC_BF16> {
  using type = bf16x8;
  static __device__ __forceinline__ type pack(float4 a, float4 b) {
    type r;
    r[0] = (__bf16)a.x; r[1] = (__bf16)a.y; r[2] = (__bf16)a.z; r[3] = (__bf16)a.w;
    r[4] = (__bf16)b.x; r[5] = (__bf16)b.y; r[6] = (__bf16)b.z; r[7] = (__bf16)b.w;
    return r;
  }
  static __device__ __forceinline__ f32x4 mfma(type a, type b, f32x4 c) {
    return __builtin_amdgcn_mfma_f32_16x16x32_bf16(a, b, c, 0, 0, 0);
  }
};
template <>
struct Frag8<PREC_F16> {
  using type = f16x8;
  static __device__ __forceinline__ type pack(float4 a, float4 b) {
    type r;
    r[0] = (_Float16)a.x; r[1] = (_Float16)a.y; r[2] = (_Float16)a.z; r[3] = (_Float16)a.w;
    r[4] = (_Float16)b.x; r[5] = (_Float16)b.y; r[6] = (_Float16)b.z; r[7] = (_Float16)b.w;
    return r;
  }
  static __device__ __forceinline__ f32x4 mfma(type a, type b, f32x4 c) {
    return __builtin_amdgcn_mfma_f32_16x16x32_f16(a, b, c, 0, 0, 0);
  }
};

__device__ __forceinline__ void wait_vmcnt(const int n) {
#define RRT_VMC(K) case K: asm volatile("s_waitcnt vmcnt(" #K ")" ::: "memory"); break;
  switch (n) {
    RRT_VMC(1) RRT_VMC(2) RRT_VMC(3) RRT_VMC(4) RRT_VMC(5) RRT_VMC(6) RRT_VMC(7) RRT_VMC(8) RRT_VMC(9) RRT_VMC(10)
    RRT_VMC(11) RRT_VMC(12) RRT_VMC(13) RRT_VMC(14) RRT_VMC(15) RRT_VMC(16) RRT_VMC(17) RRT_VMC(18) RRT_VMC(19) RRT_VMC(20)
    RRT_VMC(21) RRT_VMC(22) RRT_VMC(23) RRT_VMC(24) RRT_VMC(25) RRT_VMC(26) RRT_VMC(27) RRT_VMC(28) RRT_VMC(29) RRT_VMC(30)
    RRT_VMC(31)
    default: asm volatile("s_waitcnt vmcnt(0)" ::: "memory"); break;
  }
#undef RRT_VMC
}

__device__ __forceinline__ void map_item(const int b, const int n_items, const int heads, int& reg, int& head) {
  const int n_regions = n_items / heads;
  const int full = (n_regions >> 3) * 8 * heads;
  if (b < full) {
    const int xcd = b & 7, idx = b >> 3;
    const int grp = idx / heads;
    reg = grp * 8 + xcd;
    head = idx - grp * heads;
  } else {
    const int rem = b - full;
    reg = (n_regions >> 3) * 8 + rem / heads;
    head = rem % heads;
  }
}

#ifdef RRT_TRACE
#define RRT_SLAB_TRACE_ARG , WaveTrace& _tr
#define RRT_SLAB_TRACE_PASS , _tr
#else
#define RRT_SLAB_TRACE_ARG
#define RRT_SLAB_TRACE_PASS
#endif
#ifndef RRT_PROJ_RQA
#define RRT_PROJ_RQA 6
#endif
template <int MT, int KM>
__device__ __forceinline__ void proj_slab(const float* __restrict__ , const float* __restrict__ O, const int n_rows,
                                          const int P, const int D, const int heads_rt, const FusedProj& pj,
                                          char* smem RRT_SLAB_TRACE_ARG) {
  constexpr int BM = 16 * MT;
  constexpr int SST = (BM + HD) * BK;
  constexpr int NA = BM / 8, NB = HD / 8;
  constexpr int LA = (NA + 3) / 4, LB = NB / 4;
  constexpr bool PREF = MT <= 9;
  constexpr int LDS_MAIN_F = (2 * (BM + BN) * BK > 3 * BM * HD ? 2 * (BM + BN) * BK : 3 * BM * HD);
  constexpr int NS = LDS_MAIN_F / SST >= 4 ? 4 : LDS_MAIN_F / SST;
  static_assert(NS >= 3 && NS * SST <= LDS_MAIN_F, "slab ring");
  const int b = (int)blockIdx.x;
  if (b < pj.lag) return;
  const int sidx = b - pj.lag;
  int reg, col;
  map_item(sidx, pj.n_items, heads_rt, reg, col);
  float* lds = (float*)smem;
  const unsigned lds_b = lds_addr_of(lds);
  const int tid = threadIdx.x;
  const int lane = tid & 63;
  const int wave = __builtin_amdgcn_readfirstlane(tid >> 6);
  const int lr = lane & 15, lg = lane >> 4;
  const int row0 = reg * P;
  const int nk = D / BK;
  RRT_TRACE_MARK();
  int* const s_abort = (int*)(smem + LDS_MAIN_F * 4 + 2048);
  if (tid == 0) {
    int spins = 0, bad = 0;
    while (__hip_atomic_load(pj.cnt + reg, __ATOMIC_RELAXED, __HIP_MEMORY_SCOPE_AGENT) < pj.wait_for) {
      __builtin_amdgcn_s_sleep(8);
      if (++spins > pj.spin_limit) { bad = 1; break; }
    }
    if (bad && pj.err != nullptr) __hip_atomic_store(pj.err, 1 + reg, __ATOMIC_RELAXED, __HIP_MEMORY_SCOPE_SYSTEM);
    *s_abort = bad;
  }
  __syncthreads();
  if (*s_abort) return;
  RRT_TRACE_MARK();
  if (wave >= 4) {
    const int lw = wave - 4;
    unsigned aoff[LA], boff[LB];
#pragma unroll
    for (int qi = 0; qi < LA; ++qi) {
      const int S = (qi * 4 + lw) * 64 + lane;
      const int row = S >> 3, p = S & 7;
      int gr = row < P ? row0 + row : row0 + P - 1;
      gr = gr < n_rows ? gr : n_rows - 1;
      aoff[qi] = (unsigned)gr * (unsigned)D * 4u + (unsigned)((p ^ ((row >> 1) & 7)) << 4);
    }
#pragma unroll
    for (int qi = 0; qi < LB; ++qi) {
      const int S = (qi * 4 + lw) * 64 + lane;
      const int row = S >> 3, p = S & 7;
      boff[qi] = (unsigned)(col * HD + row) * (unsigned)D * 4u + (unsigned)((p ^ ((row >> 1) & 7)) << 4);
    }
    auto stage = [&](int kt, unsigned buf) {
#pragma unroll
      for (int qi = 0; qi < LA; ++qi)
        if (qi * 4 + lw < NA) dma16s(O + kt * BK, aoff[qi], buf + (qi * 4 + lw) * 1024);
#pragma unroll
      for (int qi = 0; qi < LB; ++qi) dma16s(pj.Wp + kt * BK, boff[qi], buf + BM * BK * 4 + (qi * 4 + lw) * 1024);
    };
    if constexpr (KM > 0) {
      float* const gpl = (float*)(smem + LDS_MAIN_F * 4);
      for (int e = tid - 256; e < 64 * KM; e += 256) {
        const int n = e >> 6, c = col * HD + (e & 63);
        gpl[e] = n < pj.k ? pj.ln_g[c] * pj.phi[(size_t)c * pj.k + n] : 0.f;
      }
    }
    const int mine = (NA - lw + 3) / 4 + LB;
    stage(0, lds_b);
    if (nk > 1) stage(1, lds_b + SST * 4);
    RRT_TRACE_MARK();
    wait_vmcnt(nk > 1 ? mine : 0);
    RRT_TRACE_MARK();
    __syncthreads();
    if (nk > 2) stage(2, lds_b + 2 * SST * 4);
    for (int kt = 0; kt < nk; ++kt) {
      wait_vmcnt(kt + 2 < nk ? mine : 0);
      if (kt == 0 || kt == 7 || kt == 14) RRT_TRACE_MARK();
      __syncthreads();
      if (kt + 3 < nk) stage(kt + 3, lds_b + ((kt + 3) % NS) * SST * 4);
    }
    return;
  }
  const int ncol = col * HD + wave * 16 + 4 * lg;
  const int tbase = [&] {
    const int ri = fdiv(reg, pj.g.rs, pj.g.inv_rs), rj = reg - ri * pj.g.rs;
    return ri * pj.g.s * pj.g.H + rj * pj.g.s;
  }();
  auto token_of = [&](const int i) {
    const int m = i * 16 + lr;
    const int pi = fdiv(m, pj.g.s, pj.g.inv_s), pjj = m - pi * pj.g.s;
    const int t = tbase + pi * pj.g.H + pjj;
    return (m < P && t < pj.g.L) ? t : -1;
  };
  int toff[MT];
#pragma unroll
  for (int i = 0; i < MT; ++i) {
    const int t = token_of(i);
    toff[i] = t < 0 ? -1 : t * D + ncol;
  }
  float4 rq[PREF ? MT : 1];
  const float4 bias = pj.bias ? *(const float4*)(pj.bias + ncol) : make_float4(0.f, 0.f, 0.f, 0.f);
  f32x4 acc[MT];
#pragma unroll
  for (int i = 0; i < MT; ++i) acc[i] = (f32x4){0.f, 0.f, 0.f, 0.f};
  float4 af[2][MT], bfr[2];
  auto frags = [&](const float* As, const int kk, float4 (&a)[MT], float4& bb) {
    {
      const int row = wave * 16 + lr;
      bb = *(const float4*)(As + BM * BK + row * BK + (((4 * kk + lg) ^ ((row >> 1) & 7)) << 2));
    }
#pragma unroll
    for (int i = 0; i < MT; ++i) {
      const int row = i * 16 + lr;
      a[i] = *(const float4*)(As + row * BK + (((4 * kk + lg) ^ ((row >> 1) & 7)) << 2));
    }
  };
  auto half = [&](const float4 (&a)[MT], const float4& bb, const bool load, const float* nAs, const int nkk,
                  float4 (&na)[MT], float4& nb) {
    if (load) frags(nAs, nkk, na, nb);
#pragma unroll
    for (int comp = 0; comp < 4; ++comp) {
      const float bv = comp == 0 ? bb.x : comp == 1 ? bb.y : comp == 2 ? bb.z : bb.w;
#pragma unroll
      for (int i = 0; i < MT; ++i) {
        const float av = comp == 0 ? a[i].x : comp == 1 ? a[i].y : comp == 2 ? a[i].z : a[i].w;
        acc[i] = __builtin_amdgcn_mfma_f32_16x16x4f32(bv, av, acc[i], 0, 0, 0);
      }
    }
    if (load) {
#pragma unroll
      for (int r = 0; r < MT + 1; ++r) {
        __builtin_amdgcn_sched_group_barrier(0x008, 3, 0);
        __builtin_amdgcn_sched_group_barrier(0x100, 1, 0);
      }
      __builtin_amdgcn_sched_group_barrier(0x008, 4 * MT - 3 * (MT + 1), 0);
    }
    __builtin_amdgcn_sched_barrier(0);
  };
  auto lds_barrier = [] { asm volatile("s_waitcnt lgkmcnt(0)\n\ts_barrier" ::: "memory"); };
  RRT_TRACE_MARK();
  lds_barrier();
  RRT_TRACE_MARK();
  frags(lds, 0, af[0], bfr[0]);
  __builtin_amdgcn_sched_barrier(0);
  auto tile = [&](const int kt) {
    half(af[0], bfr[0], true, lds + (kt % NS) * SST, 1, af[1], bfr[1]);
    lds_barrier();
    if (kt == 0 || kt == 7 || kt == 14) RRT_TRACE_MARK();
    half(af[1], bfr[1], true, lds + ((kt + 1) % NS) * SST, 0, af[0], bfr[0]);
  };
  constexpr int RQA = PREF ? (RRT_PROJ_RQA < MT ? RRT_PROJ_RQA : MT) : 0;
  for (int kt = 0; kt + 2 < nk; ++kt) tile(kt);
  if constexpr (PREF) {
#pragma unroll
    for (int i = 0; i < RQA; ++i) rq[i] = ld_row<NT_RESID>(pj.resid + (toff[i] < 0 ? ncol : toff[i]));
  }
  if (nk >= 2) tile(nk - 2);
  if constexpr (PREF) {
#pragma unroll
    for (int i = RQA; i < MT; ++i) rq[i] = ld_row<NT_RESID>(pj.resid + (toff[i] < 0 ? ncol : toff[i]));
  }
  half(af[0], bfr[0], true, lds + ((nk - 1) % NS) * SST, 1, af[1], bfr[1]);
  lds_barrier();
  half(af[1], bfr[1], false, nullptr, 0, af[0], bfr[0]);
  RRT_TRACE_MARK();
  if constexpr (PREF) {
#pragma unroll
    for (int i = 0; i < MT; ++i) asm volatile("" : "+v"(rq[i].x), "+v"(rq[i].y), "+v"(rq[i].z), "+v"(rq[i].w));
  }
  if constexpr (KM == 0) {
#pragma unroll
    for (int i = 0; i < MT; ++i) {
      float4 q;
      if constexpr (PREF) q = rq[i];
      else q = ld_row<NT_RESID>(pj.resid + (toff[i] < 0 ? ncol : toff[i]));
      const float4 v = make_float4(acc[i][0] + bias.x + q.x, acc[i][1] + bias.y + q.y, acc[i][2] + bias.z + q.z, acc[i][3] + bias.w + q.w);
      if (toff[i] >= 0) *(float4*)(pj.out + toff[i]) = v;
    }
    RRT_TRACE_MARK();
  } else {
    constexpr int NF = KM <= 2 ? 1 : KM <= 6 ? 2 : 3;
    float4* const rec = (float4*)lds;
    const float* gpl = (const float*)(smem + LDS_MAIN_F * 4);
    float4 gp[KM];
#pragma unroll
    for (int n = 0; n < KM; ++n) gp[n] = *(const float4*)(gpl + n * 64 + wave * 16 + 4 * lg);
#pragma unroll
    for (int i = 0; i < MT; ++i) {
      float4 q;
      if constexpr (PREF) q = rq[i];
      else q = ld_row<NT_RESID>(pj.resid + (toff[i] < 0 ? ncol : toff[i]));
      const float4 v = make_float4(acc[i][0] + bias.x + q.x, acc[i][1] + bias.y + q.y, acc[i][2] + bias.z + q.z, acc[i][3] + bias.w + q.w);
      if (toff[i] >= 0) *(float4*)(pj.out + toff[i]) = v;
      const float m = ((v.x + v.y) + (v.z + v.w)) * 0.25f;
      const float a = v.x - m, b = v.y - m, c = v.z - m, d = v.w - m;
      float o[4 * NF];
      o[0] = m;
      o[1] = (a * a + b * b) + (c * c + d * d);
#pragma unroll
      for (int n = 0; n < 4 * NF - 2; ++n)
        o[2 + n] = n < KM ? (v.x * gp[n < KM ? n : 0].x + v.y * gp[n < KM ? n : 0].y) + (v.z * gp[n < KM ? n : 0].z + v.w * gp[n < KM ? n : 0].w) : 0.f;
      float4* const r = rec + ((size_t)(wave * 4 + lg) * BM + i * 16 + lr) * NF;
#pragma unroll
      for (int f = 0; f < NF; ++f) r[f] = make_float4(o[4 * f], o[4 * f + 1], o[4 * f + 2], o[4 * f + 3]);
    }
    RRT_TRACE_MARK();
    lds_barrier();
    const int m_ = tid;
    if (m_ < P) {
      const int pi = fdiv(m_, pj.g.s, pj.g.inv_s), pjj = m_ - pi * pj.g.s;
      const int t = tbase + pi * pj.g.H + pjj;
      if (t < pj.g.L) {
        float o[4 * NF];
        {
          const float4* r0 = rec + (size_t)m_ * NF;
#pragma unroll
          for (int f = 0; f < NF; ++f) {
            const float4 x = r0[f];
            o[4 * f] = x.x; o[4 * f + 1] = x.y; o[4 * f + 2] = x.z; o[4 * f + 3] = x.w;
          }
        }
#pragma unroll
        for (int j = 1; j < 16; ++j) {
          const float4* rj = rec + ((size_t)j * BM + m_) * NF;
          float x[4 * NF];
#pragma unroll
          for (int f = 0; f < NF; ++f) {
            const float4 y = rj[f];
            x[4 * f] = y.x; x[4 * f + 1] = y.y; x[4 * f + 2] = y.z; x[4 * f + 3] = y.w;
          }
          const float dl = x[0] - o[0], w = 1.0f / (float)(j + 1);
          o[0] += dl * w;
          o[1] += x[1] + dl * dl * (4.0f * (float)j * w);
#pragma unroll
          for (int n = 2; n < 4 * NF; ++n) o[n] += x[n];
        }
        const int nf = (2 + pj.k + 3) >> 2;
        float4* dst = (float4*)(pj.part + ((size_t)t * pj.n_slabs + col) * (4 * nf));
        dst[0] = make_float4(o[0], o[1], o[2], o[3]);
        if constexpr (NF > 1) if (nf > 1) dst[1] = make_float4(o[4], o[5], o[6], o[7]);
        if constexpr (NF > 2) if (nf > 2) dst[2] = make_float4(o[8], o[9], o[10], o[11]);
      }
    }
    RRT_TRACE_MARK();
  }
}

template <int MT, int PREC, bool PROJ, int KM = 0>
__global__ __launch_bounds__(512, 1) void rmsa_fused_kernel(const float* __restrict__ U,
                                                            const float* __restrict__ Wqkv,
                                                            const float* __restrict__ bqkv,
                                                            const float* __restrict__ pe_w,
                                                            float* __restrict__ O, int n_rows, int P,
                                                            int D, int heads_rt, int epeg_k, float q_scale,
                                                            float* __restrict__ stash, FusedProj pj) {
  static_assert(!PROJ || PREC == PREC_F32, "the projection phase is fp32 only");
  constexpr int BM = 16 * MT;
  constexpr int STAGE = (BM + BN) * BK;
  constexpr int TILE = BM * HD;
  constexpr int NA = BM / 8, NB = BN / 8;
  constexpr int LA = (NA + 3) / 4, LB = NB / 4;
  constexpr int NT = 3;
  constexpr int LDS_MAIN = (2 * STAGE > 3 * TILE ? 2 * STAGE : 3 * TILE) * 4;
  constexpr bool PIPE = PREC == PREC_F32 && MT <= 11;
  constexpr bool SPLIT_LAST = MT == 9;
  constexpr int RUN = (BM * 16 + 511) / 512;
  constexpr int TAP_OFF = 12 + RUN - 1;
  extern __shared__ __attribute__((aligned(16))) char smem[];
  float* lds = (float*)smem;
  float* Qs = lds;
  float* Ks = lds + TILE;
  float* Vs = lds + 2 * TILE;
  float* Qt = Qs;

  const int tid = threadIdx.x;
  const int lane = tid & 63;
  const int wave = __builtin_amdgcn_readfirstlane(tid >> 6);
  const int lr = lane & 15, lg = lane >> 4;
  const unsigned lds_b = lds_addr_of(lds);
#ifndef RRT_FUSED_PRIO
#define RRT_FUSED_PRIO 3
#endif
  if (RRT_FUSED_PRIO > 0) __builtin_amdgcn_s_setprio(RRT_FUSED_PRIO);
  const int n_items = PROJ ? pj.n_items : (int)gridDim.x;
  auto item_of = [&](const int b, int& reg_, int& head_) { map_item(b, n_items, heads_rt, reg_, head_); };
  const bool has_item = !PROJ || (int)blockIdx.x < n_items;
  int head = 0, reg = 0;
  if (has_item) item_of(blockIdx.x, reg, head);
  if constexpr (PROJ) {
    if (pj.zero64 != nullptr && blockIdx.x == 0 && threadIdx.x < 64) pj.zero64[threadIdx.x] = 0;
  }
  const int row0 = reg * P;
  const int nk = D / BK;
  RRT_TRACE_INIT(blockIdx.x * 8 + wave);
  if (has_item) {
  float* const taps = (float*)(smem + LDS_MAIN);
  float* const bias_l = taps + 128;
  if (tid >= 128 && tid < 128 + BN) {
    const int n = tid - 128;
    bias_l[n] = bqkv ? bqkv[(n >> 6) * D + head * HD + (n & 63)] : 0.f;
  }
  if (tid < 128) {
    const int t = tid - TAP_OFF;
    float wt = (pe_w != nullptr && t >= 0 && t < epeg_k) ? pe_w[head * epeg_k + t] : 0.f;
    if (t == (epeg_k >> 1)) wt += 1.0f;
    taps[tid] = wt * LOG2E;
  }
  RRT_TRACE_MARK();

  if (wave >= 4) {
    const int lw = wave - 4;
    unsigned aoff[LA], boff[LB];
#pragma unroll
    for (int qi = 0; qi < LA; ++qi) {
      int S = (qi * 4 + lw) * 64 + lane;
      int row = S >> 3, p = S & 7;
      int gr = row0 + row;
      gr = gr < n_rows ? gr : n_rows - 1;
      aoff[qi] = (unsigned)gr * (unsigned)D * 4u + (unsigned)((p ^ ((row >> 1) & 7)) << 4);
    }
#pragma unroll
    for (int qi = 0; qi < LB; ++qi) {
      int S = (qi * 4 + lw) * 64 + lane;
      int row = S >> 3, p = S & 7;
      int wr = (row >> 6) * D + head * HD + (row & 63);
      boff[qi] = (unsigned)wr * (unsigned)D * 4u + (unsigned)((p ^ ((row >> 1) & 7)) << 4);
    }
    auto stage = [&](int kt, unsigned buf) {
#pragma unroll
      for (int qi = 0; qi < LA; ++qi)
        if (qi * 4 + lw < NA) dma16s(U + kt * BK, aoff[qi], buf + (qi * 4 + lw) * 1024);
#pragma unroll
      for (int qi = 0; qi < LB; ++qi) dma16s(Wqkv + kt * BK, boff[qi], buf + BM * BK * 4 + (qi * 4 + lw) * 1024);
    };
    stage(0, lds_b);
    if constexpr (PIPE) {
      wait_vm0();
      __syncthreads();
      if (nk > 1) stage(1, lds_b + STAGE * 4);
      for (int kt = 0; kt < nk; ++kt) {
        wait_vm0();
        __syncthreads();
        if (kt + 2 < nk) stage(kt + 2, lds_b + (kt & 1) * STAGE * 4);
      }
    } else {
      for (int kt = 0; kt < nk; ++kt) {
        wait_vm0();
        __syncthreads();
        if (kt + 1 < nk) stage(kt + 1, lds_b + ((kt + 1) & 1) * STAGE * 4);
      }
    }
  } else {
    f32x4 acc[MT][NT];
#pragma unroll
    for (int i = 0; i < MT; ++i)
#pragma unroll
      for (int j = 0; j < NT; ++j) acc[i][j] = (f32x4){0.f, 0.f, 0.f, 0.f};
    if constexpr (PIPE) {
      float4 af[MT], bfr[2][NT];
      auto a_frag = [&](const float* As, int kk, int i) {
        const int row = i * 16 + lr;
        return *(const float4*)(As + row * BK + (((4 * kk + lg) ^ ((row >> 1) & 7)) << 2));
      };
      auto b_frag = [&](const float* As, int kk, int j) {
        const int row = wave * (16 * NT) + j * 16 + lr;
        return *(const float4*)(As + BM * BK + row * BK + (((4 * kk + lg) ^ ((row >> 1) & 7)) << 2));
      };
      auto mm = [&](const int i, const float4 (&bc)[NT]) {
#pragma unroll
        for (int comp = 0; comp < 4; ++comp)
#pragma unroll
          for (int j = 0; j < NT; ++j) {
            const float a = comp == 0 ? af[i].x : comp == 1 ? af[i].y : comp == 2 ? af[i].z : af[i].w;
            const float b = comp == 0 ? bc[j].x : comp == 1 ? bc[j].y : comp == 2 ? bc[j].z : bc[j].w;
            acc[i][j] = __builtin_amdgcn_mfma_f32_16x16x4f32(b, a, acc[i][j], 0, 0, 0);
          }
        __builtin_amdgcn_sched_barrier(0);
      };
      auto first_half = [&](const float* As, const bool owe) {
        mm(0, bfr[0]);
        if (owe) af[MT - 1] = a_frag(As, 0, MT - 1);
        __builtin_amdgcn_sched_barrier(0);
#pragma unroll
        for (int i = 1; i < MT; ++i) {
          mm(i, bfr[0]);
          af[i - 1] = a_frag(As, 1, i - 1);
          if (i <= NT) bfr[1][i - 1] = b_frag(As, 1, i - 1);
          __builtin_amdgcn_sched_barrier(0);
        }
      };
      auto second_head = [&](const float* As) {
        mm(0, bfr[1]);
        af[MT - 1] = a_frag(As, 1, MT - 1);
        __builtin_amdgcn_sched_barrier(0);
        mm(1, bfr[1]);
      };
      auto second_tail = [&](const float* nAs, const bool refill) {
        if (refill) {
          af[0] = a_frag(nAs, 0, 0);
          bfr[0][0] = b_frag(nAs, 0, 0);
          __builtin_amdgcn_sched_barrier(0);
        }
#pragma unroll
        for (int i = 2; i < MT; ++i) {
          mm(i, bfr[1]);
          if (refill) {
            af[i - 1] = a_frag(nAs, 0, i - 1);
            if (i <= NT) bfr[0][i - 1] = b_frag(nAs, 0, i - 1);
            __builtin_amdgcn_sched_barrier(0);
          }
        }
      };
      static_assert(MT > NT, "the refill schedule needs more row tiles than column tiles");
      __syncthreads();
      RRT_TRACE_MARK();
#pragma unroll
      for (int i = 0; i < MT; ++i) af[i] = a_frag(lds, 0, i);
#pragma unroll
      for (int j = 0; j < NT; ++j) bfr[0][j] = b_frag(lds, 0, j);
      first_half(lds, false);
      second_head(lds);
      __syncthreads();
      RRT_TRACE_MARK();
      for (int kt = 1; kt < nk; ++kt) {
        const float* As = lds + (kt & 1) * STAGE;
        __builtin_amdgcn_sched_barrier(0);
        second_tail(As, true);
        first_half(As, true);
        second_head(As);
        __syncthreads();
        if (kt == 7) RRT_TRACE_MARK();
      }
      second_tail(nullptr, false);
    } else {
    for (int kt = 0; kt < nk; ++kt) {
      __syncthreads();
      if (kt == 0 || kt == 1 || kt == 8) RRT_TRACE_MARK();
      const float* As = lds + (kt & 1) * STAGE;
      const float* Bs = As + BM * BK;
      if constexpr (PREC == PREC_F32) {
#pragma unroll
        for (int kk = 0; kk < 2; ++kk) {
          float4 af[MT], bf[NT];
          const int cslot = 4 * kk + lg;
#pragma unroll
          for (int j = 0; j < NT; ++j) {
            int row = wave * (16 * NT) + j * 16 + lr;
            bf[j] = *(const float4*)(Bs + row * BK + ((cslot ^ ((row >> 1) & 7)) << 2));
          }
#pragma unroll
          for (int i = 0; i < MT; ++i) {
            int row = i * 16 + lr;
            af[i] = *(const float4*)(As + row * BK + ((cslot ^ ((row >> 1) & 7)) << 2));
          }
#pragma unroll
          for (int comp = 0; comp < 4; ++comp)
#pragma unroll
            for (int i = 0; i < MT; ++i)
#pragma unroll
              for (int j = 0; j < NT; ++j) {
                const float a = comp == 0 ? af[i].x : comp == 1 ? af[i].y : comp == 2 ? af[i].z : af[i].w;
                const float b = comp == 0 ? bf[j].x : comp == 1 ? bf[j].y : comp == 2 ? bf[j].z : bf[j].w;
                acc[i][j] = __builtin_amdgcn_mfma_f32_16x16x4f32(b, a, acc[i][j], 0, 0, 0);
              }
        }
      } else {
        using F = Frag8<PREC>;
        typename F::type a8[MT], b8[NT];
#pragma unroll
        for (int j = 0; j < NT; ++j) {
          const int row = wave * (16 * NT) + j * 16 + lr, f = (row >> 1) & 7;
          b8[j] = F::pack(*(const float4*)(Bs + row * BK + (((2 * lg) ^ f) << 2)),
                          *(const float4*)(Bs + row * BK + (((2 * lg + 1) ^ f) << 2)));
        }
#pragma unroll
        for (int i = 0; i < MT; ++i) {
          const int row = i * 16 + lr, f = (row >> 1) & 7;
          a8[i] = F::pack(*(const float4*)(As + row * BK + (((2 * lg) ^ f) << 2)),
                          *(const float4*)(As + row * BK + (((2 * lg + 1) ^ f) << 2)));
        }
#pragma unroll
        for (int i = 0; i < MT; ++i)
#pragma unroll
          for (int j = 0; j < NT; ++j) acc[i][j] = F::mfma(b8[j], a8[i], acc[i][j]);
      }
    }
    }
    RRT_TRACE_MARK();
    __syncthreads();
#pragma unroll
    for (int j = 0; j < NT; ++j) {
      const int n = wave * (16 * NT) + j * 16 + 4 * lg;
      const int c = n >> 6, d = n & 63;
      const float4 b = *(const float4*)(bias_l + n);
      const float sc = c == 0 ? q_scale : 1.0f;
      float* dstm = c == 0 ? Qs : (c == 1 ? Ks : Vs);
#pragma unroll
      for (int i = 0; i < MT; ++i) {
        const int m = i * 16 + lr;
        const int slot = (d >> 2) ^ (m & 15);
        float4 v = make_float4((acc[i][j][0] + b.x) * sc, (acc[i][j][1] + b.y) * sc,
                               (acc[i][j][2] + b.z) * sc, (acc[i][j][3] + b.w) * sc);
        *(float4*)(dstm + m * HD + (slot << 2)) = v;
      }
    }
  }
  if (wave >= 4) __syncthreads();
  __syncthreads();
  RRT_TRACE_MARK();
  if (stash != nullptr) {
    for (int idx = tid; idx < BM * 16 * 3; idx += 512) {
      const int c = idx / (BM * 16), rem = idx - c * (BM * 16);
      const int m = rem >> 4, sl = rem & 15;
      if (m < P) {
        const float4 v = *(const float4*)(lds + c * TILE + m * HD + ((sl ^ (m & 15)) << 2));
        *(float4*)(stash + (size_t)(row0 + m) * (3 * D) + c * D + head * HD + 4 * sl) = v;
// ... 7 lines not shown
    const int s = tid & 15, g = tid >> 4;
    const int r0 = g * RUN;
    f32x2 out[RUN][2];
#pragma unroll
    for (int o = 0; o < RUN; ++o) out[o][0] = out[o][1] = (f32x2){0.f, 0.f};
    if (r0 < BM) {
      const int nsrc = RUN + 2 * half;
      constexpr int NTV = (RUN + 3 + 3) / 4;
      const float4* tp4 = (const float4*)(taps + TAP_OFF - (RUN - 1));
      constexpr int NFAST = RUN + 14;
      if (nsrc <= NFAST) {
        constexpr int NTT = (NFAST + RUN - 1 + 3) / 4;
        float4 v[NFAST];
        float T[4 * NTT];
#pragma unroll
        for (int u = 0; u < NFAST; ++u) {
          const int rr = r0 - half + u;
          const bool ok = rr >= 0 && rr < P;
          const int rc = ok ? rr : 0;
          v[u] = *(const float4*)(Qs + rc * HD + ((s ^ (rc & 15)) << 2));
          if (!ok) v[u] = make_float4(0.f, 0.f, 0.f, 0.f);
        }
#pragma unroll
        for (int q = 0; q < NTT; ++q) {
          const float4 t4 = tp4[q];
          T[4 * q] = t4.x; T[4 * q + 1] = t4.y; T[4 * q + 2] = t4.z; T[4 * q + 3] = t4.w;
        }
#pragma unroll
        for (int u = 0; u < NFAST; ++u) {
          const f32x2 lo = {v[u].x, v[u].y}, hi = {v[u].z, v[u].w};
#pragma unroll
          for (int o = 0; o < RUN; ++o) {
            const float wt = T[u + RUN - 1 - o];
            const f32x2 w2 = {wt, wt};
            out[o][0] = __builtin_elementwise_fma(w2, lo, out[o][0]);
            out[o][1] = __builtin_elementwise_fma(w2, hi, out[o][1]);
          }
        }
      } else
      for (int j0 = 0; j0 < nsrc; j0 += 4) {
        float4 v[4];
        float T[4 * NTV];
#pragma unroll
        for (int q = 0; q < NTV; ++q) {
          const float4 t4 = tp4[(j0 >> 2) + q];
          T[4 * q] = t4.x; T[4 * q + 1] = t4.y; T[4 * q + 2] = t4.z; T[4 * q + 3] = t4.w;
        }
#pragma unroll
        for (int u = 0; u < 4; ++u) {
          const int rr = r0 - half + j0 + u;
          const bool ok = rr >= 0 && rr < P;
          const int rc = ok ? rr : 0;
          v[u] = *(const float4*)(Qs + rc * HD + ((s ^ (rc & 15)) << 2));
          if (!ok) v[u] = make_float4(0.f, 0.f, 0.f, 0.f);
        }
#pragma unroll
        for (int u = 0; u < 4; ++u) {
          const f32x2 lo = {v[u].x, v[u].y}, hi = {v[u].z, v[u].w};
#pragma unroll
          for (int o = 0; o < RUN; ++o) {
            const float wt = T[u + RUN - 1 - o];
            const f32x2 w2 = {wt, wt};
            out[o][0] = __builtin_elementwise_fma(w2, lo, out[o][0]);
            out[o][1] = __builtin_elementwise_fma(w2, hi, out[o][1]);
          }
        }
      }
    }
    __syncthreads();
    if (r0 < BM) {
#pragma unroll
      for (int o = 0; o < RUN; ++o) {
        const int m = r0 + o;
        if (m < BM)
          *(float4*)(Qt + m * HD + ((s ^ (m & 15)) << 2)) = make_float4(out[o][0][0], out[o][0][1], out[o][1][0], out[o][1][1]);
      }
    }
  }
  __syncthreads();
  RRT_TRACE_MARK();

  if constexpr (SPLIT_LAST) {
    constexpr int XT = MT - 1;
    float* const pstat = (float*)(smem + LDS_MAIN + 1280);
    float* const plast = pstat + MT * 32;
    const int i0 = wave * 16;
    int tk[MT];
#pragma unroll
    for (int j = 0; j < MT; ++j) tk[j] = j + wave < MT ? j + wave : j + wave - MT;
    float4 bq[4], bx[4];
    {
      const int m = i0 + lr, mx = XT * 16 + lr;
#pragma unroll
      for (int c = 0; c < 4; ++c) {
        bq[c] = *(const float4*)(Qt + m * HD + (((4 * c + lg) ^ lr) << 2));
        bx[c] = *(const float4*)(Qt + mx * HD + (((4 * c + lg) ^ lr) << 2));
      }
    }
    f32x4 s[MT], sx = {0.f, 0.f, 0.f, 0.f}, sy = {0.f, 0.f, 0.f, 0.f};
#pragma unroll
    for (int j = 0; j < MT; ++j) s[j] = (f32x4){0.f, 0.f, 0.f, 0.f};
#pragma unroll
    for (int c = 0; c < 4; ++c) {
      float4 a[MT];
#pragma unroll
      for (int j = 0; j < MT; ++j) a[j] = *(const float4*)(Ks + (tk[j] * 16 + lr) * HD + (((4 * c + lg) ^ lr) << 2));
#pragma unroll
      for (int comp = 0; comp < 4; ++comp) {
        const float qb = comp == 0 ? bq[c].x : comp == 1 ? bq[c].y : comp == 2 ? bq[c].z : bq[c].w;
        const float xb = comp == 0 ? bx[c].x : comp == 1 ? bx[c].y : comp == 2 ? bx[c].z : bx[c].w;
#pragma unroll
        for (int j = 0; j < MT; ++j) {
          const float ka = comp == 0 ? a[j].x : comp == 1 ? a[j].y : comp == 2 ? a[j].z : a[j].w;
          s[j] = __builtin_amdgcn_mfma_f32_16x16x4f32(ka, qb, s[j], 0, 0, 0);
          if (j == 0) sx = __builtin_amdgcn_mfma_f32_16x16x4f32(ka, xb, sx, 0, 0, 0);
        }
      }
    }
    if (wave == 0) {
#pragma unroll
      for (int c = 0; c < 4; ++c) {
        const float4 a8 = *(const float4*)(Ks + (XT * 16 + lr) * HD + (((4 * c + lg) ^ lr) << 2));
        sy = __builtin_amdgcn_mfma_f32_16x16x4f32(a8.x, bx[c].x, sy, 0, 0, 0);
        sy = __builtin_amdgcn_mfma_f32_16x16x4f32(a8.y, bx[c].y, sy, 0, 0, 0);
        sy = __builtin_amdgcn_mfma_f32_16x16x4f32(a8.z, bx[c].z, sy, 0, 0, 0);
        sy = __builtin_amdgcn_mfma_f32_16x16x4f32(a8.w, bx[c].w, sy, 0, 0, 0);
      }
    }
    RRT_TRACE_MARK();
    float cmax = NEG_BIG, xmax = NEG_BIG, ymax = NEG_BIG;
    if (P < BM) {
#pragma unroll
      for (int j = 0; j < MT; ++j)
#pragma unroll
        for (int r = 0; r < 4; ++r)
          if (tk[j] * 16 + 4 * lg + r >= P) s[j][r] = NEG_BIG;
#pragma unroll
      for (int r = 0; r < 4; ++r) {
        if (tk[0] * 16 + 4 * lg + r >= P) sx[r] = NEG_BIG;
        if (XT * 16 + 4 * lg + r >= P) sy[r] = NEG_BIG;
      }
    }
#pragma unroll
    for (int j = 0; j < MT; ++j)
#pragma unroll
      for (int r = 0; r < 4; ++r) cmax = fmaxf(cmax, s[j][r]);
#pragma unroll
    for (int r = 0; r < 4; ++r) {
      xmax = fmaxf(xmax, sx[r]);
      ymax = fmaxf(ymax, sy[r]);
    }
    cmax = max_xor32(max_xor16(cmax));
    xmax = max_xor32(max_xor16(xmax));
    ymax = max_xor32(max_xor16(ymax));
    float a4[4] = {0.f, 0.f, 0.f, 0.f};
#pragma unroll
    for (int j = 0; j < MT; ++j)
#pragma unroll
      for (int r = 0; r < 4; ++r) {
        const float e = __builtin_amdgcn_exp2f(s[j][r] - cmax);
        s[j][r] = e;
        a4[r] += e;
      }
    float psum = (a4[0] + a4[1]) + (a4[2] + a4[3]), xsum = 0.f, ysum = 0.f;
#pragma unroll
    for (int r = 0; r < 4; ++r) {
      sx[r] = __builtin_amdgcn_exp2f(sx[r] - xmax);
      sy[r] = __builtin_amdgcn_exp2f(sy[r] - ymax);
      xsum += sx[r];
      ysum += sy[r];
    }
    psum = sum_xor32(sum_xor16(psum));
    xsum = sum_xor32(sum_xor16(xsum));
    ysum = sum_xor32(sum_xor16(ysum));
    float ir[4];
    {
      const float inv = 1.0f / psum;
#pragma unroll
      for (int r = 0; r < 4; ++r) ir[r] = __shfl(inv, 4 * lg + r);
    }
    RRT_TRACE_MARK();
    f32x4 oacc[4], ox[4], oy[4];
#pragma unroll
    for (int c = 0; c < 4; ++c) oacc[c] = ox[c] = oy[c] = (f32x4){0.f, 0.f, 0.f, 0.f};
    {
      constexpr int G = 4 * MT, PD = 5;
      float4 vq[G];
      auto vload = [&](int g) {
        const int rr = 4 * lg + (g & 3);
        return *(const float4*)(Vs + (tk[g >> 2] * 16 + rr) * HD + ((lr ^ rr) << 2));
      };
#pragma unroll
      for (int g = 0; g < PD; ++g) vq[g] = vload(g);
#pragma unroll
      for (int g = 0; g < G; ++g) {
        __builtin_amdgcn_sched_barrier(0);
        if (g + PD < G) vq[g + PD] = vload(g + PD);
        const float4 v = vq[g];
        const float p = s[g >> 2][g & 3];
        oacc[0] = __builtin_amdgcn_mfma_f32_16x16x4f32(p, v.x, oacc[0], 0, 0, 0);
        oacc[1] = __builtin_amdgcn_mfma_f32_16x16x4f32(p, v.y, oacc[1], 0, 0, 0);
        oacc[2] = __builtin_amdgcn_mfma_f32_16x16x4f32(p, v.z, oacc[2], 0, 0, 0);
        oacc[3] = __builtin_amdgcn_mfma_f32_16x16x4f32(p, v.w, oacc[3], 0, 0, 0);
        if (g < 4) {
          const float px = sx[g];
          ox[0] = __builtin_amdgcn_mfma_f32_16x16x4f32(px, v.x, ox[0], 0, 0, 0);
          ox[1] = __builtin_amdgcn_mfma_f32_16x16x4f32(px, v.y, ox[1], 0, 0, 0);
          ox[2] = __builtin_amdgcn_mfma_f32_16x16x4f32(px, v.z, ox[2], 0, 0, 0);
          ox[3] = __builtin_amdgcn_mfma_f32_16x16x4f32(px, v.w, ox[3], 0, 0, 0);
        }
      }
      __builtin_amdgcn_sched_barrier(0);
    }
    if (wave == 0) {
#pragma unroll
      for (int r = 0; r < 4; ++r) {
        const int rr = 4 * lg + r;
        const float4 v = *(const float4*)(Vs + (XT * 16 + rr) * HD + ((lr ^ rr) << 2));
        const float py = sy[r];
        oy[0] = __builtin_amdgcn_mfma_f32_16x16x4f32(py, v.x, oy[0], 0, 0, 0);
        oy[1] = __builtin_amdgcn_mfma_f32_16x16x4f32(py, v.y, oy[1], 0, 0, 0);
        oy[2] = __builtin_amdgcn_mfma_f32_16x16x4f32(py, v.z, oy[2], 0, 0, 0);
        oy[3] = __builtin_amdgcn_mfma_f32_16x16x4f32(py, v.w, oy[3], 0, 0, 0);
      }
    }
    RRT_TRACE_MARK();
#pragma unroll
    for (int r = 0; r < 4; ++r) {
      const int i = i0 + 4 * lg + r;
      if (i < P)
        RRT_STORE_O((f32x4*)(O + (size_t)(row0 + i) * D + head * HD + (lr << 2)),
                    ((f32x4){oacc[0][r] * ir[r], oacc[1][r] * ir[r], oacc[2][r] * ir[r], oacc[3][r] * ir[r]}));
    }
    {
      float* mine = Qt + wave * 16 * HD;
#pragma unroll
      for (int r = 0; r < 4; ++r)
        *(float4*)(mine + (4 * lg + r) * HD + 4 * lr) = make_float4(ox[0][r], ox[1][r], ox[2][r], ox[3][r]);
      if (lg == 0) {
        pstat[wave * 32 + lr] = xmax;
        pstat[wave * 32 + 16 + lr] = xsum;
      }
      if (wave == 0) {
#pragma unroll
        for (int r = 0; r < 4; ++r)
          *(float4*)(plast + (4 * lg + r) * HD + 4 * lr) = make_float4(oy[0][r], oy[1][r], oy[2][r], oy[3][r]);
        if (lg == 0) {
          pstat[XT * 32 + lr] = ymax;
          pstat[XT * 32 + 16 + lr] = ysum;
        }
      }
    }
    RRT_TRACE_MARK();
    __syncthreads();
    RRT_TRACE_MARK();
    {
      const int q = tid >> 5, col = (tid & 31) * 2;
      float mw[MT], M = NEG_BIG;
#pragma unroll
      for (int w = 0; w < MT; ++w) {
        mw[w] = pstat[w * 32 + q];
        M = fmaxf(M, mw[w]);
      }
      float L = 0.f, o0 = 0.f, o1 = 0.f;
#pragma unroll
      for (int w = 0; w < MT; ++w) {
        const float sc = __builtin_amdgcn_exp2f(mw[w] - M);
        L += sc * pstat[w * 32 + 16 + q];
        const float2 a = *(const float2*)((w < XT ? Qt + w * 16 * HD : plast) + q * HD + col);
        o0 += sc * a.x;
        o1 += sc * a.y;
      }
      const float invL = 1.0f / L;
      if (XT * 16 + q < P)
        RRT_STORE_O((f32x2*)(O + (size_t)(row0 + XT * 16 + q) * D + head * HD + col), ((f32x2){o0 * invL, o1 * invL}));
      RRT_TRACE_MARK();
    }
  } else {
  for (int t = wave; t < MT; t += 8) {
    const int i0 = t * 16;
    if (i0 >= P) break;
    float4 bq[4];
    {
      const int m = i0 + lr;
#pragma unroll
      for (int c = 0; c < 4; ++c) bq[c] = *(const float4*)(Qt + m * HD + (((4 * c + lg) ^ (m & 15)) << 2));
    }
    f32x4 s[MT];
#pragma unroll
    for (int jt = 0; jt < MT; ++jt) s[jt] = (f32x4){0.f, 0.f, 0.f, 0.f};
#pragma unroll
    for (int c = 0; c < 4; ++c) {
      float4 a[MT];
#pragma unroll
      for (int jt = 0; jt < MT; ++jt) {
        const int row = jt * 16 + lr;
        a[jt] = *(const float4*)(Ks + row * HD + (((4 * c + lg) ^ (row & 15)) << 2));
      }
#pragma unroll
      for (int jt = 0; jt < MT; ++jt) s[jt] = __builtin_amdgcn_mfma_f32_16x16x4f32(a[jt].x, bq[c].x, s[jt], 0, 0, 0);
#pragma unroll
      for (int jt = 0; jt < MT; ++jt) s[jt] = __builtin_amdgcn_mfma_f32_16x16x4f32(a[jt].y, bq[c].y, s[jt], 0, 0, 0);
#pragma unroll
      for (int jt = 0; jt < MT; ++jt) s[jt] = __builtin_amdgcn_mfma_f32_16x16x4f32(a[jt].z, bq[c].z, s[jt], 0, 0, 0);
#pragma unroll
      for (int jt = 0; jt < MT; ++jt) s[jt] = __builtin_amdgcn_mfma_f32_16x16x4f32(a[jt].w, bq[c].w, s[jt], 0, 0, 0);
    }
    RRT_TRACE_MARK();
    float cmax = NEG_BIG;
    if (P < BM) {
#pragma unroll
      for (int jt = 0; jt < MT; ++jt)
#pragma unroll
        for (int r = 0; r < 4; ++r)
          if (jt * 16 + 4 * lg + r >= P) s[jt][r] = NEG_BIG;
    }
#pragma unroll
    for (int jt = 0; jt < MT; ++jt)
#pragma unroll
      for (int r = 0; r < 4; ++r) cmax = fmaxf(cmax, s[jt][r]);
    cmax = max_xor32(max_xor16(cmax));
    float a4[4] = {0.f, 0.f, 0.f, 0.f};
#pragma unroll
    for (int jt = 0; jt < MT; ++jt)
#pragma unroll
      for (int r = 0; r < 4; ++r) {
        const float e = __builtin_amdgcn_exp2f(s[jt][r] - cmax);
        s[jt][r] = e;
        a4[r] += e;
      }
    const float psum = sum_xor32(sum_xor16((a4[0] + a4[1]) + (a4[2] + a4[3])));
    float ir[4];
    {
      const float inv = 1.0f / psum;
#pragma unroll
      for (int r = 0; r < 4; ++r) ir[r] = __shfl(inv, 4 * lg + r);
    }
    RRT_TRACE_MARK();
    f32x4 oacc[4];
#pragma unroll
    for (int c = 0; c < 4; ++c) oacc[c] = (f32x4){0.f, 0.f, 0.f, 0.f};
#pragma unroll
    for (int jt = 0; jt < MT; ++jt)
#pragma unroll
      for (int r = 0; r < 4; ++r) {
        const int row = jt * 16 + 4 * lg + r;
        const float4 v = *(const float4*)(Vs + row * HD + ((lr ^ (row & 15)) << 2));
        const float p = s[jt][r];
        oacc[0] = __builtin_amdgcn_mfma_f32_16x16x4f32(p, v.x, oacc[0], 0, 0, 0);
        oacc[1] = __builtin_amdgcn_mfma_f32_16x16x4f32(p, v.y, oacc[1], 0, 0, 0);
        oacc[2] = __builtin_amdgcn_mfma_f32_16x16x4f32(p, v.z, oacc[2], 0, 0, 0);
        oacc[3] = __builtin_amdgcn_mfma_f32_16x16x4f32(p, v.w, oacc[3], 0, 0, 0);
      }
    RRT_TRACE_MARK();
#pragma unroll
    for (int r = 0; r < 4; ++r) {
      const int i = i0 + 4 * lg + r;
      if (i < P)
        RRT_STORE_O((f32x4*)(O + (size_t)(row0 + i) * D + head * HD + (lr << 2)),
                    ((f32x4){oacc[0][r] * ir[r], oacc[1][r] * ir[r], oacc[2][r] * ir[r], oacc[3][r] * ir[r]}));
    }
    RRT_TRACE_MARK();
  }
  }
  if constexpr (PROJ) {
    wait_vm0();
    __syncthreads();
    RRT_TRACE_MARK();
    if (tid == 0) __hip_atomic_fetch_add(pj.cnt + reg, 1, __ATOMIC_RELAXED, __HIP_MEMORY_SCOPE_AGENT);
  }
  }
  if constexpr (PROJ) proj_slab<MT, KM>(U, O, n_rows, P, D, heads_rt, pj, smem RRT_SLAB_TRACE_PASS);
}

int proj_lag(int n_items) {
  static int cus[64] = {};
  int d = 0;
  (void)hipGetDevice(&d);
  d &= 63;
  if (cus[d] == 0) {
    int n = 0;
    if (hipDeviceGetAttribute(&n, hipDeviceAttributeMultiprocessorCount, d) != hipSuccess || n <= 0) n = 256;
    cus[d] = n;
  }
  int lag = cus[d] & ~7;
  if (lag > n_items) lag = n_items & ~7;
  static const char* force = rrt_tune_env("RRT_PROJ_LAG");
  if (force != nullptr && atoi(force) > 0) lag = atoi(force);
  return lag;
}

template <int MT, int PREC>
hipError_t launch_mt(const float* U, const float* Wqkv, const float* bqkv, const float* pe_w, float* O,
                     int n_regions, int P, int D, int heads, int epeg_k, float* stash, hipStream_t st,
                     const FusedProj* proj) {
  constexpr int BM = 16 * MT;
  constexpr size_t STG = (size_t)2 * (BM + BN) * BK * 4, QKV = (size_t)3 * BM * HD * 4;
  constexpr size_t LDS = (STG > QKV ? STG : QKV) + (MT == 9 ? 1280 + MT * 32 * 4 + 16 * HD * 4 : 2064);
  static_assert(LDS <= 160 * 1024, "LDS budget");
  const float q_scale = 1.0f / sqrtf((float)HD);
  if constexpr (PREC == PREC_F32) {
    if (proj != nullptr) {
      FusedProj pj = *proj;
      pj.n_items = heads * n_regions;
      if (pj.lag <= 0) pj.lag = proj_lag(pj.n_items);
      if (pj.wait_for <= 0) pj.wait_for = heads;
      pj.n_slabs = D / HD;
      if (pj.part != nullptr && (pj.ln_g == nullptr || pj.phi == nullptr || pj.k < 1 || pj.k > RRT_MAX_CRMSA_K))
        return hipErrorInvalidValue;
      if (pj.spin_limit <= 0) pj.spin_limit = 1 << 22;
      if (pj.err == nullptr) pj.err = handover_err_device();
#define RRT_LAUNCH_PROJ(KM_)                                                                                    \
  do {                                                                                                           \
    auto kern = rmsa_fused_kernel<MT, PREC_F32, true, KM_>;                                                      \
    static OncePerDevice once;                                                                                   \
    if (once.first())                                                                                            \
      (void)hipFuncSetAttribute((const void*)kern, hipFuncAttributeMaxDynamicSharedMemorySize, (int)LDS);        \
    kern<<<dim3(pj.n_items + pj.lag), dim3(512), LDS, st>>>(U, Wqkv, bqkv, pe_w, O, n_regions * P, P, D, heads,  \
                                                            pe_w ? epeg_k : 0, q_scale, nullptr, pj);            \
  } while (0)
      if constexpr (MT >= 6) {
        if (pj.part != nullptr && pj.k <= 4) RRT_LAUNCH_PROJ(4);
        else if (pj.part != nullptr) RRT_LAUNCH_PROJ(8);
        else RRT_LAUNCH_PROJ(0);
      } else {
        if (pj.part != nullptr) return hipErrorInvalidValue;
        RRT_LAUNCH_PROJ(0);
      }
#undef RRT_LAUNCH_PROJ
      return hipGetLastError();
    }
  }
  auto kern = rmsa_fused_kernel<MT, PREC, false>;
  static OncePerDevice once;
  if (once.first())
    (void)hipFuncSetAttribute((const void*)kern, hipFuncAttributeMaxDynamicSharedMemorySize, (int)LDS);
  kern<<<dim3(heads * n_regions), dim3(512), LDS, st>>>(U, Wqkv, bqkv, pe_w, O, n_regions * P, P, D, heads,
                                                      pe_w ? epeg_k : 0, q_scale, stash, FusedProj{});
  return hipGetLastError();
}

}

#ifdef RRT_TRACE
RRT_TRACE_DEFINE_READER(rrt_debug_trace_fused)
// ... 71 lines not shown
```

Before: 5467.

## Skip padded row tiles in fused RMSA+projection for edge regions

Computes per region how many 16-row tiles actually contain real tokens (edge regions are padded when L is not a square grid) and dispatches templated variants of the QKV GEMM, attention, and projection slab with fewer row tiles. Padded query tiles are skipped in attention and projection, which removes MFMA work and loads on padding rows. It is on by default when padding exists and can be disabled with an environment variable. In exchange it adds code size through many template instantiations and divergent per-block work, and only the MT=9 and MT=11 configurations get it.

Measured after the change: 5464. About the same (-0.0%).

```diff
diff --git a/include/rrt_hip.h b/include/rrt_hip.h
--- a/include/rrt_hip.h
+++ b/include/rrt_hip.h
@@ -98,6 +98,7 @@
 #define RRT_PLAN_ATTN_HD    32
 int rrt_encoder_plan(const rrt_encoder_desc *desc, int64_t n_tokens, int32_t *flags);
 int rrt_encoder_plan_rows(const rrt_encoder_desc *desc, int64_t n_tokens, int32_t *w);
+int rrt_encoder_plan_pad_tiles(const rrt_encoder_desc *desc, int64_t n_tokens, int32_t *skip);
 
 int rrt_encoder_forward_f32(const rrt_encoder_desc *desc, const rrt_encoder_weights *w,
                             const float *x, float *y, int64_t n_tokens,
@@ -106,6 +107,10 @@
 int rrt_debug_encoder_forward_rows_f32(const rrt_encoder_desc *desc, const rrt_encoder_weights *w,
                                        const float *x, float *y, int64_t n_tokens,
                                        void *workspace, size_t workspace_bytes, void *stream, int32_t rows_w);
+
+int rrt_debug_encoder_forward_pad_tiles_f32(const rrt_encoder_desc *desc, const rrt_encoder_weights *w,
+                                            const float *x, float *y, int64_t n_tokens,
+                                            void *workspace, size_t workspace_bytes, void *stream, int32_t mode);
 
 enum {
   RRT_EV_START = 0,
@@ -195,6 +200,11 @@
                                   const float *proj_w, const float *proj_b, const float *resid, float *out,
                                   float *o_scratch, int32_t *counters, int32_t dim, int32_t heads, int32_t epeg_k,
                                   const rrt_grid *g, int32_t lag, int32_t spin_limit, int32_t wait_extra, void *stream);
+int rrt_debug_rmsa_fused_proj_pad_tiles_f32(const float *u, const float *qkv_w, const float *qkv_b, const float *pe_w,
+                                            const float *proj_w, const float *proj_b, const float *resid, float *out,
+                                            float *o_scratch, int32_t *counters, const float *ln2_gamma, const float *phi,
+                                            int32_t crmsa_k, float *part, int32_t dim, int32_t heads, int32_t epeg_k,
+                                            const rrt_grid *g, int32_t skip_pad, void *stream);
 
 int rrt_cast16(const float *src, uint16_t *dst, int64_t n, int32_t compute, void *stream);
 int rrt_ln_partition16(const float *x, const float *gamma, const float *beta, uint16_t *u, int64_t L,
diff --git a/rrt-mil_amd/_lib.py b/rrt-mil_amd/_lib.py
--- a/rrt-mil_amd/_lib.py
+++ b/rrt-mil_amd/_lib.py
@@ -163,6 +163,9 @@
     "rrt_encoder_workspace_size": (C.c_int, [C.POINTER(EncoderDesc), C.c_int64, C.POINTER(C.c_size_t)]),
     "rrt_encoder_plan": (C.c_int, [C.POINTER(EncoderDesc), C.c_int64, C.POINTER(C.c_int32)]),
     "rrt_encoder_plan_rows": (C.c_int, [C.POINTER(EncoderDesc), C.c_int64, C.POINTER(C.c_int32)]),
+    "rrt_encoder_plan_pad_tiles": (C.c_int, [C.POINTER(EncoderDesc), C.c_int64, C.POINTER(C.c_int32)]),
+    "rrt_debug_encoder_forward_pad_tiles_f32": (C.c_int, [C.POINTER(EncoderDesc), C.POINTER(EncoderWeights), C.c_void_p,
+                                                          C.c_void_p, C.c_int64, C.c_void_p, C.c_size_t, C.c_void_p, C.c_int32]),
     "rrt_encoder_forward_f32": (C.c_int, [C.POINTER(EncoderDesc), C.POINTER(EncoderWeights), C.c_void_p,
                                           C.c_void_p, C.c_int64, C.c_void_p, C.c_size_t, C.c_void_p]),
     "rrt_debug_encoder_forward_rows_f32": (C.c_int, [C.POINTER(EncoderDesc), C.POINTER(EncoderWeights), C.c_void_p,
@@ -203,6 +206,8 @@
     "rrt_rmsa_fused_proj_stats_f32": (C.c_int, [C.c_void_p] * 12 + [C.c_int32, C.c_void_p] + [C.c_int32] * 3 + [C.c_void_p] * 2),
     "rrt_crmsa_combine_parts_f32": (C.c_int, [C.c_void_p] * 7 + [C.c_int64, C.c_int32, C.c_int32, C.POINTER(Grid), C.c_void_p]),
     "rrt_debug_rmsa_fused_proj_f32": (C.c_int, [C.c_void_p] * 10 + [C.c_int32] * 3 + [C.c_void_p] + [C.c_int32] * 3 + [C.c_void_p]),
+    "rrt_debug_rmsa_fused_proj_pad_tiles_f32": (C.c_int, [C.c_void_p] * 12 + [C.c_int32, C.c_void_p] + [C.c_int32] * 3 +
+                                                [C.c_void_p, C.c_int32, C.c_void_p]),
     "rrt_cast16": (C.c_int, [C.c_void_p, C.c_void_p, C.c_int64, C.c_int32, C.c_void_p]),
     "rrt_ln_partition16": (C.c_int, [C.c_void_p, C.c_void_p, C.c_void_p, C.c_void_p, C.c_int64, C.c_int32,
                                      C.POINTER(Grid), C.c_int32, C.c_void_p]),
diff --git a/rrt-mil_amd/csrc/api.hip b/rrt-mil_amd/csrc/api.hip
--- a/rrt-mil_amd/csrc/api.hip
+++ b/rrt-mil_amd/csrc/api.hip
@@ -213,6 +213,7 @@
   FrontKind front;
   int rows_w;
   bool rows_ln1;
+  bool skip_pad;
 };
 
 constexpr int ROWS_W_DEFAULT = 1;
@@ -255,6 +256,8 @@
       p.layer = LayerKind::FusedX3;
     } else if (compute == RRT_COMPUTE_F32 && rows_ok && rmsa_fused_proj_supported(R, gd.P, D, heads, ek, compute)) {
       p.layer = LayerKind::FusedProj;
+      static const bool no_pad_skip = rrt_tune_env("RRT_NO_PAD_SKIP") != nullptr;
+      p.skip_pad = !no_pad_skip && g.add > 0;
       p.parts = d.solo != 0 && d.cr_msa && !d.crmsa_mlp && !d.ffn && d.crmsa_k <= 4 && !stops_before_crmsa && D % 64 == 0 &&
                 crmsa_combine_parts_supported(D, d.crmsa_k, gd8);
     } else if (rmsa_fused_supported(gd.P, D, heads, ek) && rows_ok) {
@@ -380,6 +383,17 @@
   return RRT_OK;
 }
 
+int rrt_encoder_plan_pad_tiles(const rrt_encoder_desc* desc, int64_t n_tokens, int32_t* skip) {
+  if (!skip) return RRT_E_INVALID;
+  *skip = 0;
+  rrt_grid g{}, g8{};
+  int rc = resolve_grids(desc, n_tokens, &g, &g8);
+  if (rc) return rc;
+  if (desc->n_rmsa_layers <= 0) return RRT_OK;
+  *skip = plan_encoder(*desc, g, g8, false).skip_pad ? 1 : 0;
+  return RRT_OK;
+}
+
 int rrt_encoder_plan_rows(const rrt_encoder_desc* desc, int64_t n_tokens, int32_t* w) {
   if (!w) return RRT_E_INVALID;
   *w = 0;
@@ -413,7 +427,7 @@
                            float* y, int64_t n_tokens, void* workspace, size_t workspace_bytes,
                            void* stream, void** events, rrt_phase_gate* gate = nullptr, float* rmsa_out = nullptr,
                            uint16_t* y16 = nullptr, bool* y16_done = nullptr, int rows_w_forced = -1,
-                           const float* shortcut = nullptr) {
+                           const float* shortcut = nullptr, int pad_tiles_forced = -1) {
   if (y16_done) *y16_done = false;
   if (!desc_in || !w || !x || !y || x == y) return RRT_E_INVALID;
   int rc = check_desc(desc_in, n_tokens);
@@ -435,6 +449,13 @@
   if (rows_w_forced >= 0) {
     plan.rows_w = rows_w_forced;
     plan.rows_ln1 = rows_w_forced > 0 && desc_in->compute == RRT_COMPUTE_F32;
+  }
+  if (pad_tiles_forced >= 0 && plan.layer == LayerKind::FusedProj) {
+    if (pad_tiles_forced == 2) {
+      if (plan.parts) return unsupported("the two-launch plan cannot be forced where CR-MSA's front reads the merged launch's row records (solo)");
+      plan.layer = LayerKind::Fused;
+    }
+    plan.skip_pad = pad_tiles_forced == 1;
   }
 
   auto mark = [&](int i) -> hipError_t {
@@ -570,6 +591,7 @@
         pj.cnt = ws.proj_cnt;
         pj.zero64 = ws.cr_cnt;
         pj.g = gd;
+        pj.skip_pad = plan.skip_pad ? 1 : 0;
         if (plan.parts && last) {
           pj.part = ws.cr_pstat;
           pj.ln_g = w->crmsa.norm_w;
@@ -724,6 +746,14 @@
   return encoder_forward(desc, w, x, y, n_tokens, workspace, workspace_bytes, stream, nullptr);
 }
 
+int rrt_debug_encoder_forward_pad_tiles_f32(const rrt_encoder_desc* desc, const rrt_encoder_weights* w, const float* x, float* y,
+                                            int64_t n_tokens, void* workspace, size_t workspace_bytes, void* stream,
+                                            int32_t mode) {
+  if (mode < 0 || mode > 2) return RRT_E_INVALID;
+  return encoder_forward(desc, w, x, y, n_tokens, workspace, workspace_bytes, stream, nullptr, nullptr, nullptr, nullptr, nullptr,
+                         -1, nullptr, mode);
+}
+
 int rrt_debug_encoder_forward_rows_f32(const rrt_encoder_desc* desc, const rrt_encoder_weights* w, const float* x, float* y,
                                        int64_t n_tokens, void* workspace, size_t workspace_bytes, void* stream, int32_t rows_w) {
   if (rows_w < 0 || rows_w > ROWS_W_MAX) return RRT_E_INVALID;
@@ -996,7 +1026,7 @@
                             const float* proj_w, const float* proj_b, const float* resid, float* out, float* o_scratch,
                             int32_t* counters, int32_t dim, int32_t heads, int32_t epeg_k, const rrt_grid* g,
                             int32_t lag, int32_t spin_limit, int32_t wait_extra, const float* ln2_gamma, const float* phi,
-                            int32_t crmsa_k, float* part, void* stream) {
+                            int32_t crmsa_k, float* part, void* stream, int32_t skip_pad = 0) {
   if (!u || !qkv_w || !proj_w || !resid || !out || !o_scratch || !counters || !g || dim <= 0 || heads <= 0 || out == resid ||
       lag < 0 || spin_limit < 0 || wait_extra < 0)
     return RRT_E_INVALID;
@@ -1021,6 +1051,7 @@
   pj.ln_g = ln2_gamma;
   pj.phi = phi;
   pj.k = crmsa_k;
+  pj.skip_pad = skip_pad != 0;
   if (lag > 0 && (lag < 8 * heads || lag > heads * R)) return unsupported("rmsa_fused_proj: lag must be in [8 * heads, heads * regions]");
   return (int)launch_rmsa_fused(u, qkv_w, qkv_b, pe_w, o_scratch, R, gd.P, dim, heads, ek, RRT_COMPUTE_F32,
                                 (hipStream_t)stream, nullptr, &pj);
@@ -1043,6 +1074,17 @@
   if (!ln2_gamma || !phi || !part || crmsa_k < 1 || crmsa_k > RRT_MAX_CRMSA_K) return RRT_E_INVALID;
   return fused_proj_stage(u, qkv_w, qkv_b, pe_w, proj_w, proj_b, resid, out, o_scratch, counters, dim, heads, epeg_k, g, 0, 0, 0,
                           ln2_gamma, phi, crmsa_k, part, stream);
+}
+
+int rrt_debug_rmsa_fused_proj_pad_tiles_f32(const float* u, const float* qkv_w, const float* qkv_b, const float* pe_w,
+                                            const float* proj_w, const float* proj_b, const float* resid, float* out,
+                                            float* o_scratch, int32_t* counters, const float* ln2_gamma, const float* phi,
+                                            int32_t crmsa_k, float* part, int32_t dim, int32_t heads, int32_t epeg_k,
+                                            const rrt_grid* g, int32_t skip_pad, void* stream) {
+  if (part != nullptr && (!ln2_gamma || !phi || crmsa_k < 1 || crmsa_k > RRT_MAX_CRMSA_K)) return RRT_E_INVALID;
+  if (skip_pad < 0 || skip_pad > 1) return RRT_E_INVALID;
+  return fused_proj_stage(u, qkv_w, qkv_b, pe_w, proj_w, proj_b, resid, out, o_scratch, counters, dim, heads, epeg_k, g, 0, 0, 0,
+                          part ? ln2_gamma : nullptr, part ? phi : nullptr, part ? crmsa_k : 0, part, stream, skip_pad);
 }
 
 int rrt_crmsa_combine_parts_f32(const float* x1, const float* part, const float* gamma, const float* beta, const float* phi,
diff --git a/rrt-mil_amd/csrc/internal.h b/rrt-mil_amd/csrc/internal.h
--- a/rrt-mil_amd/csrc/internal.h
+++ b/rrt-mil_amd/csrc/internal.h
@@ -139,6 +139,7 @@
   const float* phi;
   int k;
   int n_slabs;
+  int skip_pad;
 };
 int* handover_err_device();
 int handover_err_peek(bool clear);
diff --git a/rrt-mil_amd/csrc/rmsa_fused.hip b/rrt-mil_amd/csrc/rmsa_fused.hip
--- a/rrt-mil_amd/csrc/rmsa_fused.hip
+++ b/rrt-mil_amd/csrc/rmsa_fused.hip
@@ -86,6 +86,27 @@
     head = rem % heads;
   }
 }
+
+__device__ __forceinline__ int eff_row_tiles(const GridDev& g, const int reg, const int mt) {
+  const int ri = fdiv(reg, g.rs, g.inv_rs), rj = reg - ri * g.rs;
+  const int last = g.L - 1 - (ri * g.s * g.H + rj * g.s);
+  const int pi = fdiv(last < 0 ? 0 : last, g.H, g.inv_H), pjj = last - pi * g.H;
+  int m = pi >= g.s ? g.P - 1 : pi * g.s + (pjj < g.s ? pjj : g.s - 1);
+  if (last < 0) m = -16;
+  const int t = (m >> 4) + 1;
+  return __builtin_amdgcn_readfirstlane(t < mt ? t : mt);
+}
+constexpr int MTE_MIN = 4;
+template <int N>
+struct RowTiles { static constexpr int value = N; };
+template <int LO, int HI, class F>
+__device__ __forceinline__ void with_row_tiles(const int n, F&& f) {
+  if constexpr (LO >= HI) f(RowTiles<HI>{});
+  else if (n >= HI) f(RowTiles<HI>{});
+  else with_row_tiles<LO, HI - 1>(n, f);
+}
+constexpr bool pad_skip_built(const int mt) { return mt == 9 || mt == 11; }
+constexpr bool pad_skip_slab_built(const int mt) { return mt == 11; }
 
 #ifdef RRT_TRACE
 #define RRT_SLAB_TRACE_ARG , WaveTrace& _tr
@@ -114,6 +135,11 @@
   const int sidx = b - pj.lag;
   int reg, col;
   map_item(sidx, pj.n_items, heads_rt, reg, col);
+  int mte = MT;
+  if constexpr (pad_skip_built(MT)) {
+    if (pj.skip_pad) mte = eff_row_tiles(pj.g, reg, MT);
+    if (mte == 0) return;
+  }
   float* lds = (float*)smem;
   const unsigned lds_b = lds_addr_of(lds);
   const int tid = threadIdx.x;
@@ -194,48 +220,51 @@
     const int t = tbase + pi * pj.g.H + pjj;
     return (m < P && t < pj.g.L) ? t : -1;
   };
-  int toff[MT];
-#pragma unroll
-  for (int i = 0; i < MT; ++i) {
+  auto compute = [&](auto me_c) {
+  constexpr int ME = decltype(me_c)::value;
+  int toff[ME];
+#pragma unroll
+  for (int i = 0; i < ME; ++i) {
     const int t = token_of(i);
     toff[i] = t < 0 ? -1 : t * D + ncol;
   }
-  float4 rq[PREF ? MT : 1];
+  float4 rq[PREF ? ME : 1];
   const float4 bias = pj.bias ? *(const float4*)(pj.bias + ncol) : make_float4(0.f, 0.f, 0.f, 0.f);
-  f32x4 acc[MT];
-#pragma unroll
-  for (int i = 0; i < MT; ++i) acc[i] = (f32x4){0.f, 0.f, 0.f, 0.f};
-  float4 af[2][MT], bfr[2];
-  auto frags = [&](const float* As, const int kk, float4 (&a)[MT], float4& bb) {
+  f32x4 acc[ME];
+#pragma unroll
+  for (int i = 0; i < ME; ++i) acc[i] = (f32x4){0.f, 0.f, 0.f, 0.f};
+  float4 af[2][ME], bfr[2];
+  auto frags = [&](const float* As, const int kk, float4 (&a)[ME], float4& bb) {
     {
       const int row = wave * 16 + lr;
       bb = *(const float4*)(As + BM * BK + row * BK + (((4 * kk + lg) ^ ((row >> 1) & 7)) << 2));
     }
 #pragma unroll
-    for (int i = 0; i < MT; ++i) {
+    for (int i = 0; i < ME; ++i) {
       const int row = i * 16 + lr;
       a[i] = *(const float4*)(As + row * BK + (((4 * kk + lg) ^ ((row >> 1) & 7)) << 2));
     }
   };
-  auto half = [&](const float4 (&a)[MT], const float4& bb, const bool load, const float* nAs, const int nkk,
-                  float4 (&na)[MT], float4& nb) {
+  static_assert(4 * ME >= 3 * (ME + 1), "read / MFMA interleave of a half K tile");
+  auto half = [&](const float4 (&a)[ME], const float4& bb, const bool load, const float* nAs, const int nkk,
+                  float4 (&na)[ME], float4& nb) {
     if (load) frags(nAs, nkk, na, nb);
 #pragma unroll
     for (int comp = 0; comp < 4; ++comp) {
       const float bv = comp == 0 ? bb.x : comp == 1 ? bb.y : comp == 2 ? bb.z : bb.w;
 #pragma unroll
-      for (int i = 0; i < MT; ++i) {
+      for (int i = 0; i < ME; ++i) {
         const float av = comp == 0 ? a[i].x : comp == 1 ? a[i].y : comp == 2 ? a[i].z : a[i].w;
         acc[i] = __builtin_amdgcn_mfma_f32_16x16x4f32(bv, av, acc[i], 0, 0, 0);
       }
     }
     if (load) {
 #pragma unroll
-      for (int r = 0; r < MT + 1; ++r) {
+      for (int r = 0; r < ME + 1; ++r) {
         __builtin_amdgcn_sched_group_barrier(0x008, 3, 0);
         __builtin_amdgcn_sched_group_barrier(0x100, 1, 0);
       }
-      __builtin_amdgcn_sched_group_barrier(0x008, 4 * MT - 3 * (MT + 1), 0);
+      __builtin_amdgcn_sched_group_barrier(0x008, 4 * ME - 3 * (ME + 1), 0);
     }
     __builtin_amdgcn_sched_barrier(0);
   };
@@ -251,7 +280,7 @@
     if (kt == 0 || kt == 7 || kt == 14) RRT_TRACE_MARK();
     half(af[1], bfr[1], true, lds + ((kt + 1) % NS) * SST, 0, af[0], bfr[0]);
   };
-  constexpr int RQA = PREF ? (RRT_PROJ_RQA < MT ? RRT_PROJ_RQA : MT) : 0;
+  constexpr int RQA = PREF ? (RRT_PROJ_RQA < ME ? RRT_PROJ_RQA : ME) : 0;
   for (int kt = 0; kt + 2 < nk; ++kt) tile(kt);
   if constexpr (PREF) {
 #pragma unroll
@@ -260,7 +289,7 @@
   if (nk >= 2) tile(nk - 2);
   if constexpr (PREF) {
 #pragma unroll
-    for (int i = RQA; i < MT; ++i) rq[i] = ld_row<NT_RESID>(pj.resid + (toff[i] < 0 ? ncol : toff[i]));
+    for (int i = RQA; i < ME; ++i) rq[i] = ld_row<NT_RESID>(pj.resid + (toff[i] < 0 ? ncol : toff[i]));
   }
   half(af[0], bfr[0], true, lds + ((nk - 1) % NS) * SST, 1, af[1], bfr[1]);
   lds_barrier();
@@ -268,11 +297,11 @@
   RRT_TRACE_MARK();
   if constexpr (PREF) {
 #pragma unroll
-    for (int i = 0; i < MT; ++i) asm volatile("" : "+v"(rq[i].x), "+v"(rq[i].y), "+v"(rq[i].z), "+v"(rq[i].w));
+    for (int i = 0; i < ME; ++i) asm volatile("" : "+v"(rq[i].x), "+v"(rq[i].y), "+v"(rq[i].z), "+v"(rq[i].w));
   }
   if constexpr (KM == 0) {
 #pragma unroll
-    for (int i = 0; i < MT; ++i) {
+    for (int i = 0; i < ME; ++i) {
       float4 q;
       if constexpr (PREF) q = rq[i];
       else q = ld_row<NT_RESID>(pj.resid + (toff[i] < 0 ? ncol : toff[i]));
@@ -288,7 +317,7 @@
 #pragma unroll
     for (int n = 0; n < KM; ++n) gp[n] = *(const float4*)(gpl + n * 64 + wave * 16 + 4 * lg);
 #pragma unroll
-    for (int i = 0; i < MT; ++i) {
+    for (int i = 0; i < ME; ++i) {
       float4 q;
       if constexpr (PREF) q = rq[i];
       else q = ld_row<NT_RESID>(pj.resid + (toff[i] < 0 ? ncol : toff[i]));
@@ -346,6 +375,14 @@
     }
     RRT_TRACE_MARK();
   }
+  };
+  if constexpr (pad_skip_slab_built(MT)) {
+    if (mte < MT) {
+      with_row_tiles<MTE_MIN, MT - 1>(mte, compute);
+      return;
+    }
+  }
+  compute(RowTiles<MT>{});
 }
 
 template <int MT, int PREC, bool PROJ, int KM = 0>
@@ -395,7 +432,12 @@
   const int row0 = reg * P;
   const int nk = D / BK;
   RRT_TRACE_INIT(blockIdx.x * 8 + wave);
+  int mte = MT;
+  if constexpr (PROJ && pad_skip_built(MT)) {
+    if (pj.skip_pad && has_item) mte = eff_row_tiles(pj.g, reg, MT);
+  }
   if (has_item) {
+  if (mte > 0) {
   float* const taps = (float*)(smem + LDS_MAIN);
   float* const bias_l = taps + 128;
   if (tid >= 128 && tid < 128 + BN) {
@@ -459,7 +501,9 @@
 #pragma unroll
       for (int j = 0; j < NT; ++j) acc[i][j] = (f32x4){0.f, 0.f, 0.f, 0.f};
     if constexpr (PIPE) {
-      float4 af[MT], bfr[2][NT];
+      auto pipe = [&](auto me_c) {
+      constexpr int ME = decltype(me_c)::value;
+      float4 af[ME], bfr[2][NT];
       auto a_frag = [&](const float* As, int kk, int i) {
         const int row = i * 16 + lr;
         return *(const float4*)(As + row * BK + (((4 * kk + lg) ^ ((row >> 1) & 7)) << 2));
@@ -481,10 +525,10 @@
       };
       auto first_half = [&](const float* As, const bool owe) {
         mm(0, bfr[0]);
-        if (owe) af[MT - 1] = a_frag(As, 0, MT - 1);
+        if (owe) af[ME - 1] = a_frag(As, 0, ME - 1);
         __builtin_amdgcn_sched_barrier(0);
 #pragma unroll
-        for (int i = 1; i < MT; ++i) {
+        for (int i = 1; i < ME; ++i) {
           mm(i, bfr[0]);
           af[i - 1] = a_frag(As, 1, i - 1);
           if (i <= NT) bfr[1][i - 1] = b_frag(As, 1, i - 1);
@@ -493,7 +537,7 @@
       };
       auto second_head = [&](const float* As) {
         mm(0, bfr[1]);
-        af[MT - 1] = a_frag(As, 1, MT - 1);
+        af[ME - 1] = a_frag(As, 1, ME - 1);
         __builtin_amdgcn_sched_barrier(0);
         mm(1, bfr[1]);
       };
@@ -504,7 +548,7 @@
           __builtin_amdgcn_sched_barrier(0);
         }
 #pragma unroll
-        for (int i = 2; i < MT; ++i) {
+        for (int i = 2; i < ME; ++i) {
           mm(i, bfr[1]);
           if (refill) {
             af[i - 1] = a_frag(nAs, 0, i - 1);
@@ -513,11 +557,11 @@
           }
         }
       };
-      static_assert(MT > NT, "the refill schedule needs more row tiles than column tiles");
+      static_assert(ME > NT, "the refill schedule needs more row tiles than column tiles");
       __syncthreads();
       RRT_TRACE_MARK();
 #pragma unroll
-      for (int i = 0; i < MT; ++i) af[i] = a_frag(lds, 0, i);
+      for (int i = 0; i < ME; ++i) af[i] = a_frag(lds, 0, i);
 #pragma unroll
       for (int j = 0; j < NT; ++j) bfr[0][j] = b_frag(lds, 0, j);
       first_half(lds, false);
@@ -534,6 +578,13 @@
         if (kt == 7) RRT_TRACE_MARK();
       }
       second_tail(nullptr, false);
+      };
+      if constexpr (PROJ && pad_skip_built(MT)) {
+        if (mte < MT) with_row_tiles<MTE_MIN, MT - 1>(mte, pipe);
+        else pipe(RowTiles<MT>{});
+      } else {
+        pipe(RowTiles<MT>{});
+      }
     } else {
     for (int kt = 0; kt < nk; ++kt) {
       __syncthreads();
@@ -707,6 +758,8 @@
 
   if constexpr (SPLIT_LAST) {
     constexpr int XT = MT - 1;
+    auto split = [&](auto x9_c) {
+    constexpr bool X9 = decltype(x9_c)::value != 0;
     float* const pstat = (float*)(smem + LDS_MAIN + 1280);
     float* const plast = pstat + MT * 32;
     const int i0 = wave * 16;
@@ -719,7 +772,7 @@
 #pragma unroll
       for (int c = 0; c < 4; ++c) {
         bq[c] = *(const float4*)(Qt + m * HD + (((4 * c + lg) ^ lr) << 2));
-        bx[c] = *(const float4*)(Qt + mx * HD + (((4 * c + lg) ^ lr) << 2));
+        if constexpr (X9) bx[c] = *(const float4*)(Qt + mx * HD + (((4 * c + lg) ^ lr) << 2));
       }
     }
     f32x4 s[MT], sx = {0.f, 0.f, 0.f, 0.f}, sy = {0.f, 0.f, 0.f, 0.f};
@@ -733,16 +786,16 @@
 #pragma unroll
       for (int comp = 0; comp < 4; ++comp) {
         const float qb = comp == 0 ? bq[c].x : comp == 1 ? bq[c].y : comp == 2 ? bq[c].z : bq[c].w;
-        const float xb = comp == 0 ? bx[c].x : comp == 1 ? bx[c].y : comp == 2 ? bx[c].z : bx[c].w;
+        const float xb = !X9 ? 0.f : comp == 0 ? bx[c].x : comp == 1 ? bx[c].y : comp == 2 ? bx[c].z : bx[c].w;
 #pragma unroll
         for (int j = 0; j < MT; ++j) {
           const float ka = comp == 0 ? a[j].x : comp == 1 ? a[j].y : comp == 2 ? a[j].z : a[j].w;
           s[j] = __builtin_amdgcn_mfma_f32_16x16x4f32(ka, qb, s[j], 0, 0, 0);
-          if (j == 0) sx = __builtin_amdgcn_mfma_f32_16x16x4f32(ka, xb, sx, 0, 0, 0);
-        }
-      }
-    }
-    if (wave == 0) {
+          if (X9 && j == 0) sx = __builtin_amdgcn_mfma_f32_16x16x4f32(ka, xb, sx, 0, 0, 0);
+        }
+      }
+    }
+    if (X9 && wave == 0) {
 #pragma unroll
       for (int c = 0; c < 4; ++c) {
         const float4 a8 = *(const float4*)(Ks + (XT * 16 + lr) * HD + (((4 * c + lg) ^ lr) << 2));
@@ -761,7 +814,7 @@
         for (int r = 0; r < 4; ++r)
           if (tk[j] * 16 + 4 * lg + r >= P) s[j][r] = NEG_BIG;
 #pragma unroll
-      for (int r = 0; r < 4; ++r) {
+      for (int r = 0; X9 && r < 4; ++r) {
         if (tk[0] * 16 + 4 * lg + r >= P) sx[r] = NEG_BIG;
         if (XT * 16 + 4 * lg + r >= P) sy[r] = NEG_BIG;
       }
@@ -771,13 +824,15 @@
 #pragma unroll
       for (int r = 0; r < 4; ++r) cmax = fmaxf(cmax, s[j][r]);
 #pragma unroll
-    for (int r = 0; r < 4; ++r) {
+    for (int r = 0; X9 && r < 4; ++r) {
       xmax = fmaxf(xmax, sx[r]);
       ymax = fmaxf(ymax, sy[r]);
     }
     cmax = max_xor32(max_xor16(cmax));
-    xmax = max_xor32(max_xor16(xmax));
-    ymax = max_xor32(max_xor16(ymax));
+    if constexpr (X9) {
+      xmax = max_xor32(max_xor16(xmax));
+      ymax = max_xor32(max_xor16(ymax));
+    }
     float a4[4] = {0.f, 0.f, 0.f, 0.f};
 #pragma unroll
     for (int j = 0; j < MT; ++j)
@@ -789,15 +844,17 @@
       }
     float psum = (a4[0] + a4[1]) + (a4[2] + a4[3]), xsum = 0.f, ysum = 0.f;
 #pragma unroll
-    for (int r = 0; r < 4; ++r) {
+    for (int r = 0; X9 && r < 4; ++r) {
       sx[r] = __builtin_amdgcn_exp2f(sx[r] - xmax);
       sy[r] = __builtin_amdgcn_exp2f(sy[r] - ymax);
       xsum += sx[r];
       ysum += sy[r];
     }
     psum = sum_xor32(sum_xor16(psum));
-    xsum = sum_xor32(sum_xor16(xsum));
-    ysum = sum_xor32(sum_xor16(ysum));
+    if constexpr (X9) {
+      xsum = sum_xor32(sum_xor16(xsum));
+      ysum = sum_xor32(sum_xor16(ysum));
+    }
     float ir[4];
     {
       const float inv = 1.0f / psum;
@@ -827,7 +884,7 @@
         oacc[1] = __builtin_amdgcn_mfma_f32_16x16x4f32(p, v.y, oacc[1], 0, 0, 0);
         oacc[2] = __builtin_amdgcn_mfma_f32_16x16x4f32(p, v.z, oacc[2], 0, 0, 0);
         oacc[3] = __builtin_amdgcn_mfma_f32_16x16x4f32(p, v.w, oacc[3], 0, 0, 0);
-        if (g < 4) {
+        if (X9 && g < 4) {
           const float px = sx[g];
           ox[0] = __builtin_amdgcn_mfma_f32_16x16x4f32(px, v.x, ox[0], 0, 0, 0);
           ox[1] = __builtin_amdgcn_mfma_f32_16x16x4f32(px, v.y, ox[1], 0, 0, 0);
@@ -837,7 +894,7 @@
       }
       __builtin_amdgcn_sched_barrier(0);
     }
-    if (wave == 0) {
+    if (X9 && wave == 0) {
 #pragma unroll
       for (int r = 0; r < 4; ++r) {
         const int rr = 4 * lg + r;
@@ -857,7 +914,7 @@
         RRT_STORE_O((f32x4*)(O + (size_t)(row0 + i) * D + head * HD + (lr << 2)),
                     ((f32x4){oacc[0][r] * ir[r], oacc[1][r] * ir[r], oacc[2][r] * ir[r], oacc[3][r] * ir[r]}));
     }
-    {
+    if constexpr (X9) {
       float* mine = Qt + wave * 16 * HD;
 #pragma unroll
       for (int r = 0; r < 4; ++r)
@@ -877,6 +934,7 @@
       }
     }
     RRT_TRACE_MARK();
+    if constexpr (X9) {
     __syncthreads();
     RRT_TRACE_MARK();
     {
@@ -901,10 +959,17 @@
         RRT_STORE_O((f32x2*)(O + (size_t)(row0 + XT * 16 + q) * D + head * HD + col), ((f32x2){o0 * invL, o1 * invL}));
       RRT_TRACE_MARK();
     }
+    }
+    };
+    if (mte >= MT) split(RowTiles<1>{});
+    else if (wave < mte) split(RowTiles<0>{});
   } else {
   for (int t = wave; t < MT; t += 8) {
     const int i0 = t * 16;
     if (i0 >= P) break;
+    if constexpr (PROJ && pad_skip_built(MT)) {
+      if (t >= mte) break;
+    }
     float4 bq[4];
     {
       const int m = i0 + lr;
@@ -986,6 +1051,7 @@
                     ((f32x4){oacc[0][r] * ir[r], oacc[1][r] * ir[r], oacc[2][r] * ir[r], oacc[3][r] * ir[r]}));
     }
     RRT_TRACE_MARK();
+  }
   }
   }
   if constexpr (PROJ) {
```
